# krzyz/topo-renderer

Measured on AMD Instinct MI355X. Metric: panorama Mpix/s, higher is better.
Workload: dtype f32; 1 GPU; c4: 10x10 deg COP90-shaped mosaic (100 tiles of 1200x1200 f32), 16384x4096 panorama = 8 sectors of 2048x4096, view_mode 0; frames_in_flight=1

## Files before the change

topo-renderer_amd/__init__.py:

```python
from __future__ import annotations

import ctypes as C
import math
import os
import subprocess

import numpy as np

from . import panorama, synth

_HERE = os.path.dirname(os.path.abspath(__file__))
LIB_PATH = os.environ.get("TOPO_HIP_LIB") or os.path.join(_HERE, "libtopo_hip.so")
HEADER_PATH = os.path.join(os.path.dirname(_HERE), "include", "topo_hip.h")
TEST_HEADER_PATH = os.path.join(os.path.dirname(_HERE), "include", "topo_hip_test.h")

TOPO_OK = 0
TOPO_ERR_INVALID, TOPO_ERR_UNSUPPORTED, TOPO_ERR_HIP, TOPO_ERR_NOT_FOUND, TOPO_ERR_CAPACITY = -1, -2, -3, -4, -5
FORMAT_RGBA8_UNORM_SRGB, FORMAT_BGRA8_UNORM_SRGB, FORMAT_RGBA8_UNORM, FORMAT_BGRA8_UNORM = 1, 2, 3, 4
TIMING_SLOTS = 9
TIMING_NAMES = ("clear", "cull", "raster", "occlusion", "raster_big", "resolve", "total", "load", "load_tables")

NEAR, FAR = 50.0, 500000.0
N_SECTORS = 8
HORIZON_SKY, HORIZON_INCOMPLETE = -1, -2
HORIZON_DTYPE = np.dtype([("row", "<i4"), ("depth", "<f4"), ("lat_deg", "<i4"), ("lon_deg", "<i4"), ("cell_x", "<u4"), ("cell_y", "<u4"),
                          ("fan", "<u4"), ("_reserved", "<u4")])
GROUND_TERRAIN, GROUND_SKY, GROUND_OUTSIDE, GROUND_INCOMPLETE, GROUND_DEGENERATE = 1, 0, -1, -2, -3
GROUND_DTYPE = np.dtype([("lon_deg", "<f8"), ("lat_deg", "<f8"), ("height_m", "<f4"), ("range_m", "<f4"), ("depth", "<f4"), ("kind", "<i4"),
                         ("tile_lat_deg", "<i4"), ("tile_lon_deg", "<i4"), ("cell_x", "<u4"), ("cell_y", "<u4"), ("tri", "<u4"), ("fan", "<u4"),
                         ("w1", "<f4"), ("w2", "<f4")])
GROUND_QUERY_DTYPE = np.dtype([("view", "<u4"), ("x", "<u4"), ("y", "<u4"), ("_reserved", "<u4")])
RAY_HIT, RAY_MISS, RAY_INVALID = 1, 0, -1
SUN_NONE, SUN_LIT, SUN_AWAY, SUN_SHADOW = 0, 1, 2, 3
RAY_DTYPE = np.dtype([("origin", "<f8", 3), ("dir", "<f8", 3), ("t_min", "<f8"), ("t_max", "<f8")])
RAY_HIT_DTYPE = np.dtype([("t", "<f8"), ("lon_deg", "<f8"), ("lat_deg", "<f8"), ("height_m", "<f4"), ("kind", "<i4"), ("tile_lat_deg", "<i4"),
                          ("tile_lon_deg", "<i4"), ("cell_x", "<u4"), ("cell_y", "<u4"), ("tri", "<u4"), ("front", "<u4"), ("w1", "<f4"), ("w2", "<f4")])
UNWRAP_EQUIRECTANGULAR, UNWRAP_CYLINDRICAL = 0, 1
UNWRAP_NEAREST, UNWRAP_BILINEAR = 0, 1
UNWRAP_PARAMS_DTYPE = np.dtype([("projection", "<u4"), ("filter", "<u4"), ("out_w", "<u4"), ("out_h", "<u4"), ("az0_deg", "<f8"), ("az_span_deg", "<f8"),
                                ("el_top_deg", "<f8"), ("el_bottom_deg", "<f8")])


class TopoError(RuntimeError):
    def __init__(self, code, msg):
        super().__init__(f"topo_hip error {code}: {msg}")
        self.code = code


def build(verbose: bool = False) -> str:
    subprocess.check_call(["make", "-C", os.path.join(_HERE, "csrc"), "all"] + ([] if verbose else ["-s"]))
    return LIB_PATH


_lib = None


def _preload_torch_hip_runtime():
    import importlib.util
    try:
        spec = importlib.util.find_spec("torch")
    except (ImportError, ValueError):
        spec = None
    if spec and spec.submodule_search_locations:
        cand = os.path.join(list(spec.submodule_search_locations)[0], "lib", "libamdhip64.so")
        if os.path.exists(cand):
            C.CDLL(cand, mode=C.RTLD_GLOBAL)


def lib():
    global _lib
    if _lib is None:
        if not os.path.exists(LIB_PATH):
            raise ImportError(f"{LIB_PATH} is missing -- run `python -c 'import __graft_entry__ as g; g.build()'` "
                              "(there is no Python/CPU fallback for the render path)")
        _preload_torch_hip_runtime()
        L = C.CDLL(LIB_PATH)
        vp, u32, i32, f32, sz = C.c_void_p, C.c_uint32, C.c_int32, C.c_float, C.c_size_t
        sigs = {
            "topo_create": (C.c_int, [C.POINTER(vp), C.c_int, u32, u32, u32]),
            "topo_destroy": (None, [vp]),
            "topo_last_error": (C.c_char_p, [vp]),
            "topo_add_terrain": (C.c_int, [vp, i32, i32, vp, u32, u32, vp, vp, vp]),
            "topo_add_terrain_device": (C.c_int, [vp, i32, i32, vp, u32, u32, vp, vp, vp]),
            "topo_unload_terrain": (C.c_int, [vp, i32, i32]),
            "topo_update": (C.c_int, [vp, u32, u32, vp, vp]),
            "topo_render": (C.c_int, [vp, vp, sz, vp, sz]),
            "topo_recompute_normals": (C.c_int, [vp]),
            "topo_render_views_device": (C.c_int, [vp, u32, vp, u32, u32, vp, sz, sz, vp, sz, sz]),
            "topo_set_stream": (C.c_int, [vp, vp]),
            "topo_synchronize": (C.c_int, [vp]),
            "topo_set_normals_lds_rows": (C.c_int, [vp, C.c_int]),
            "topo_debug_set_queue_caps": (C.c_int, [vp, u32, u32]),
            "topo_debug_far_phase_launched": (C.c_int, [vp, vp]),
            "topo_debug_set_tile_prefilter": (C.c_int, [vp, i32]),
            "topo_debug_cull_pairs": (C.c_int, [vp, vp]),
            "topo_pin_host_buffer": (C.c_int, [vp, vp, sz]),
            "topo_unpin_host_buffer": (C.c_int, [vp, vp]),
            "topo_get_timings": (C.c_int, [vp, vp]),
            "topo_get_timing_history": (C.c_int, [vp, C.c_uint32, vp, vp]),
            "topo_get_counters": (C.c_int, [vp, vp]),
            "topo_set_occlusion_split": (C.c_int, [vp, f32]),
            "topo_set_timing_slots": (C.c_int, [vp, u32]),
            "topo_read_normals": (C.c_int, [vp, i32, i32, vp]),
            "topo_read_tile_tables": (C.c_int, [vp, i32, i32, vp, vp, vp, vp]),
            "topo_probe_sincos": (C.c_int, [vp, vp, vp, vp, sz]),
            "topo_probe_div": (C.c_int, [vp, i32, vp, vp, vp, sz]),
            "topo_set_pipeline_depth": (C.c_int, [vp, i32]),
            "topo_join": (C.c_int, [vp]),
            "topo_frame_status": (C.c_int, [vp, vp]),
            "topo_overlay_lines": (C.c_int, [vp, vp, u32, vp, u32, f32, vp, sz]),
            "topo_overlay_lines_device": (C.c_int, [vp, vp, u32, vp, u32, f32, vp, sz]),
            "topo_overlay_glyphs": (C.c_int, [vp, vp, u32, C.c_float, vp, u32, u32, vp, sz]),
            "topo_overlay_glyphs_device": (C.c_int, [vp, vp, u32, C.c_float, vp, u32, u32, vp, sz]),
            "topo_change_location_plan": (None, [f32, f32, f32, vp, u32, vp, u32, vp, vp, u32, vp]),
            "topo_change_location": (C.c_int, [vp, f32, f32, f32, vp, u32, vp, vp]),
            "topo_comm_unique_id": (C.c_int, [vp]),
            "topo_comm_init": (C.c_int, [C.POINTER(vp), C.c_int, vp, C.c_int, C.c_int]),
            "topo_comm_from_nccl": (C.c_int, [C.POINTER(vp), vp, C.c_int, C.c_int]),
            "topo_comm_destroy": (None, [vp]),
            "topo_panorama_sector_range": (None, [C.c_int, C.c_int, vp, vp]),
            "topo_panorama_slots": (u32, [C.c_int, u32, u32, vp, u32]),
            "topo_render_panorama": (C.c_int, [vp, vp, vp, f32, f32, u32, u32, f32, f32, i32, vp, vp]),
            "topo_render_batch": (C.c_int, [vp, u32, vp, vp, vp, f32, u32, u32, i32, vp, vp]),
            "topo_visible_peaks": (C.c_int, [vp, u32, vp, vp, vp]),
            "topo_visible_peaks_device": (C.c_int, [vp, vp, u32, u32, vp, sz, u32, vp, vp, vp]),
            "topo_camera_uniforms": (None, [vp, f32, f32, f32, f32, f32, f32, f32, i32, vp]),
            "topo_terrain_uniforms": (None, [vp, vp, vp, u32, u32, vp]),
            "topo_geometry_transform": (None, [f32, f32, f32, vp]),
            "topo_dist_from_depth": (f32, [f32]),
            "topo_pad_256": (u32, [u32]),
            "topo_synth_tile": (None, [i32, i32, u32, u32, u32, vp]),
            "topo_locations_range": (u32, [f32, f32, f32, vp, u32]),
            "topo_coordinate_transform": (C.c_int, [vp, u32, vp, u32, vp, vp, vp, vp]),
            "topo_geotiff_info": (C.c_int, [vp, sz, vp, vp, vp, vp, vp]),
            "topo_sector_fov_y": (f32, [u32, u32, u32]),
            "topo_panorama_uniforms": (None, [vp, f32, f32, u32, u32, f32, f32, i32, u32, vp]),
            "topo_render_device": (C.c_int, [vp, vp, sz, vp, sz]),
            "topo_geotiff_decode": (C.c_int, [vp, vp, sz, vp, sz]),
            "topo_add_terrain_geotiff": (C.c_int, [vp, i32, i32, vp, sz]),
            "topo_to_model": (None, [vp, vp, vp, f32, f32, vp]),
            "topo_to_raster": (None, [vp, vp, vp, f32, f32, vp]),
            "topo_height_value_at": (C.c_int, [vp, u32, u32, vp, vp, vp, C.c_double, C.c_double, vp]),
            "topo_viewshed_enable": (C.c_int, [vp, i32]),
            "topo_viewshed_reset": (C.c_int, [vp]),
            "topo_viewshed_read": (C.c_int, [vp, i32, i32, vp, sz, vp]),
            "topo_debug_viewshed_stats": (C.c_int, [vp, vp]),
            "topo_horizon_shape": (C.c_int, [vp, vp, vp, vp]),
            "topo_horizon_read": (C.c_int, [vp, u32, u32, vp, sz]),
            "topo_horizon_device": (C.c_int, [vp, u32, u32, vp, sz]),
            "topo_pixel_angles": (None, [vp, u32, u32, u32, vp, vp]),
            "topo_ground_read": (C.c_int, [vp, u32, vp, vp]),
            "topo_ground_device": (C.c_int, [vp, u32, vp, vp]),
            "topo_ground_map_device": (C.c_int, [vp, u32, u32, vp, sz, sz]),
            "topo_raycast_read": (C.c_int, [vp, u32, vp, vp]),
            "topo_raycast_device": (C.c_int, [vp, u32, vp, vp]),
            "topo_sunlit_map_device": (C.c_int, [vp, u32, u32, vp, vp, sz, sz]),
            "topo_sun_direction": (None, [C.c_double, C.c_double, C.c_double, C.c_double, vp]),
            "topo_unwrap_device": (C.c_int, [vp, vp, u32, vp, u32, u32, vp, sz, sz, vp, sz, sz, vp, sz, vp, sz, vp, sz]),
            "topo_unwrap_xy": (None, [vp, u32, vp, vp]),
        }
        for name, (res, args) in sigs.items():
            fn = getattr(L, name)
            fn.restype = res
            fn.argtypes = args
        L._topo_symbols = tuple(sigs)
        _lib = L
    return _lib


def _p(a):
    return a.ctypes.data_as(C.c_void_p)



def camera_uniforms(eye, yaw, pitch, fov_y, width, height, sun_theta_deg, sun_phi_deg, view_mode=0) -> np.ndarray:
    out = np.zeros(40, dtype=np.float32)
    e = np.ascontiguousarray(eye, dtype=np.float32)
    lib().topo_camera_uniforms(_p(e), yaw, pitch, fov_y, width, height, sun_theta_deg, sun_phi_deg, view_mode, _p(out))
# ... 305 lines not shown

    def overlay_glyphs(self, glyphs, atlas: np.ndarray, rgba: np.ndarray, depth: float = 100.0 / 4096.0) -> np.ndarray:
        g = np.ascontiguousarray(glyphs)
        a = np.ascontiguousarray(atlas, dtype=np.uint8)
        assert rgba.dtype == np.uint8 and rgba.flags.c_contiguous
        self._check(lib().topo_overlay_glyphs(self._h, _p(g), g.nbytes // 28, depth, _p(a), a.shape[1], a.shape[0], _p(rgba), rgba.strides[0]))
        return rgba

    def overlay_glyphs_device(self, glyphs, atlas: np.ndarray, rgba_ptr: int, rgba_pitch: int, depth: float = 100.0 / 4096.0):
        g = np.ascontiguousarray(glyphs)
        a = np.ascontiguousarray(atlas, dtype=np.uint8)
        self._check(lib().topo_overlay_glyphs_device(self._h, _p(g), g.nbytes // 28, depth, _p(a), a.shape[1], a.shape[0], C.c_void_p(rgba_ptr), rgba_pitch))

    def change_location(self, latitude: float, longitude: float, range_dist: float = 100_000.0):
        rq = np.zeros((4096, 2), np.int32)
        nr, nu = C.c_uint32(), C.c_uint32()
        self._check(lib().topo_change_location(self._h, latitude, longitude, range_dist, _p(rq), 4096, C.byref(nr), C.byref(nu)))
        return [(int(a), int(b)) for a, b in rq[:nr.value]], int(nu.value)

    def render_panorama(self, comm, eye, yaw0, sector_w, sector_h, sun_theta_deg, sun_phi_deg, strip_ptr: int, depth_ptr: int = 0,
                        view_mode: int = 0, pitch: float = 0.0):
        e = np.ascontiguousarray(eye, dtype=np.float32)
        self._check(lib().topo_render_panorama(self._h, comm._h if comm is not None else None, _p(e), yaw0, pitch, sector_w, sector_h,
                                               sun_theta_deg, sun_phi_deg, view_mode, C.c_void_p(strip_ptr),
                                               C.c_void_p(depth_ptr) if depth_ptr else None))

    def render_batch(self, eyes, yaw0s, suns_theta_phi_deg, sector_w, sector_h, rgba_ptr: int, depth_ptr: int = 0, view_mode: int = 0,
                     pitch: float = 0.0):
        e = np.ascontiguousarray(eyes, dtype=np.float32).reshape(-1, 3)
        y = np.ascontiguousarray(yaw0s, dtype=np.float32).reshape(-1)
        sn = np.ascontiguousarray(suns_theta_phi_deg, dtype=np.float32).reshape(-1, 2)
        assert len(e) == len(y) == len(sn)
        self._check(lib().topo_render_batch(self._h, len(e), _p(e), _p(y), _p(sn), pitch, sector_w, sector_h, view_mode,
                                            C.c_void_p(rgba_ptr), C.c_void_p(depth_ptr) if depth_ptr else None))

    def render_views_device(self, uniforms_list, width, height, rgba_ptr: int, rgba_view_stride: int, rgba_pitch: int,
                            depth_ptr: int = 0, depth_view_stride: int = 0, depth_pitch: int = 0):
        if isinstance(uniforms_list, np.ndarray) and uniforms_list.dtype == np.uint8 and uniforms_list.ndim == 2:
            us = np.ascontiguousarray(uniforms_list)
            assert us.shape[1] == 160
        else:
            us = np.ascontiguousarray(np.stack([np.ascontiguousarray(u).view(np.uint8).reshape(160) for u in uniforms_list]))
        self._check(lib().topo_render_views_device(self._h, len(us), _p(us), width, height,
                                                   C.c_void_p(rgba_ptr), rgba_view_stride, rgba_pitch,
                                                   C.c_void_p(depth_ptr) if depth_ptr else None, depth_view_stride, depth_pitch))

    def set_stream(self, hip_stream: int):
        self._check(lib().topo_set_stream(self._h, C.c_void_p(hip_stream) if hip_stream else None))

    def set_pipeline_depth(self, depth: int):
        self._check(lib().topo_set_pipeline_depth(self._h, depth))

    def join(self):
        self._check(lib().topo_join(self._h))

    def synchronize(self):
        self._check(lib().topo_synchronize(self._h))

    def frame_status(self) -> dict:
        out = np.zeros(4, np.uint32)
        self._check(lib().topo_frame_status(self._h, _p(out)))
        return {"status": int(out[0]), "big_overflow": bool(out[0] & 1), "rare_overflow": bool(out[0] & 2), "bounds_violation": bool(out[0] & 4),
                "bounds_site": int(out[1]), "bounds_value": int(out[2]) | (int(out[3]) << 32)}

    def set_normals_lds_rows(self, rows: int):
        self._check(lib().topo_set_normals_lds_rows(self._h, rows))

    def debug_set_queue_caps(self, big_cap: int, rare_cap: int):
        self._check(lib().topo_debug_set_queue_caps(self._h, big_cap, rare_cap))

    def debug_far_phase_launched(self) -> bool:
        out = np.zeros(1, np.int32)
        self._check(lib().topo_debug_far_phase_launched(self._h, _p(out)))
        return bool(out[0])

    def debug_set_tile_prefilter(self, on: bool):
        self._check(lib().topo_debug_set_tile_prefilter(self._h, 1 if on else 0))

    def debug_cull_pairs(self) -> tuple:
        out = np.zeros(2, np.uint32)
        self._check(lib().topo_debug_cull_pairs(self._h, _p(out)))
        return int(out[0]), int(out[1])

    def timings(self) -> dict:
        out = np.zeros(TIMING_SLOTS, np.float32)
        self._check(lib().topo_get_timings(self._h, _p(out)))
        return {k: float(v) for k, v in zip(TIMING_NAMES, out) if k != "_"}

    def timing_history(self, n_frames: int) -> list:
        out, n = np.zeros((max(1, n_frames), 7), np.float32), C.c_uint32(0)
        self._check(lib().topo_get_timing_history(self._h, n_frames, _p(out), C.byref(n)))
        return [{k: float(v) for k, v in zip(TIMING_NAMES[:7], row)} for row in out[:n.value]]

    def counters(self) -> dict:
        out = np.zeros(6, np.uint32)
        self._check(lib().topo_get_counters(self._h, _p(out)))
        return {"blocks_rastered": int(out[0]) + int(out[5]), "big_items": int(out[1]), "status": int(out[2]), "rare_items": int(out[3]),
                "near_blocks": int(out[0]), "far_tested": int(out[4]), "far_survived": int(out[5])}

    def set_timing_slots(self, names=None, total=True):
        mask = 0x3F if names is None else sum(1 << TIMING_NAMES.index(n) for n in names)
        if not total:
            mask |= 0x80
        self._check(lib().topo_set_timing_slots(self._h, mask))

    def set_occlusion_split(self, metres: float):
        self._check(lib().topo_set_occlusion_split(self._h, metres))

    def read_tile_tables(self, lat_deg, lon_deg) -> dict:
        w, h = self.tile_size
        n = C.c_uint32(0)
        self._check(lib().topo_read_tile_tables(self._h, lat_deg, lon_deg, None, None, None, C.byref(n)))
        minmax, trig, bounds = np.empty((n.value, 2), np.float32), np.empty((w + h, 2), np.float32), np.empty(n.value * 17, np.float64)
        self._check(lib().topo_read_tile_tables(self._h, lat_deg, lon_deg, _p(minmax), _p(trig), _p(bounds), C.byref(n)))
        return {"minmax": minmax, "trig": trig, "bounds": bounds}

    def read_normals(self, lat_deg, lon_deg) -> np.ndarray:
        w, h = self.tile_size
        out = np.empty((h, w, 4), np.uint8)
        self._check(lib().topo_read_normals(self._h, lat_deg, lon_deg, _p(out)))
        return out

    def visible_peaks(self, peaks_xyz: np.ndarray):
        pk = np.ascontiguousarray(peaks_xyz, dtype=np.float32).reshape(-1, 3)
        n = pk.shape[0]
        vis = np.zeros(n, np.uint8)
        xy = np.zeros((n, 2), np.uint32)
        self._check(lib().topo_visible_peaks(self._h, n, _p(pk), _p(vis), _p(xy)))
        return vis.astype(bool), xy

    def visible_peaks_device(self, uniforms, width, height, depth_ptr, depth_pitch, n, peaks_ptr, visible_ptr, xy_ptr):
        u = np.ascontiguousarray(uniforms).view(np.uint8)
        self._check(lib().topo_visible_peaks_device(self._h, _p(u), width, height, C.c_void_p(depth_ptr), depth_pitch, n,
                                                    C.c_void_p(peaks_ptr), C.c_void_p(visible_ptr), C.c_void_p(xy_ptr)))

    def viewshed_enable(self, on: bool = True):
        self._check(lib().topo_viewshed_enable(self._h, 1 if on else 0))

    def viewshed_reset(self):
        self._check(lib().topo_viewshed_reset(self._h))

    def viewshed(self, lat_deg, lon_deg) -> np.ndarray:
        if self.tile_size is None:
            raise TopoError(TOPO_ERR_NOT_FOUND, "no tile loaded")
        w, h = self.tile_size
        out = np.zeros((h - 1, w - 1), np.uint8)
        n = C.c_uint64(0)
        self._check(lib().topo_viewshed_read(self._h, lat_deg, lon_deg, _p(out), w - 1, C.byref(n)))
        if int(out.sum()) != n.value:
            raise TopoError(TOPO_ERR_INVALID, f"viewshed count {n.value} differs from the mask's {int(out.sum())} cells")
        return out.astype(bool)

    def debug_viewshed_stats(self) -> dict:
        out = np.zeros(3, np.uint64)
        self._check(lib().topo_debug_viewshed_stats(self._h, _p(out)))
        return {"terrain_keys": int(out[0]), "updates": int(out[1]), "atomics": int(out[2])}

    def horizon_shape(self):
        n, w, h = C.c_uint32(), C.c_uint32(), C.c_uint32()
        self._check(lib().topo_horizon_shape(self._h, C.byref(n), C.byref(w), C.byref(h)))
        return int(n.value), int(w.value), int(h.value)

    def horizon(self, first_view: int = 0, n_views: int = None) -> np.ndarray:
        total, w, _ = self.horizon_shape()
        n = total - first_view if n_views is None else n_views
        out = np.zeros((max(n, 0), w), HORIZON_DTYPE)
# ... 69 lines not shown
```

topo-renderer_amd/csrc/kernels_frame.h:

```cpp
#pragma once

#include "kernels_common.h"

namespace topo {
namespace {

__device__ __forceinline__ void clear_body(uint64_t* __restrict__ vis, uint8_t* __restrict__ dirty, size_t n, uint32_t* __restrict__ counters,
                                           uint32_t* __restrict__ zero, uint32_t block, uint32_t n_blocks) {
    if (block == 0)
        for (uint32_t i = threadIdx.x; i < kCounterWords; i += 256) zero[i] = 0;
    const uint32_t lane = threadIdx.x & 63;
    const size_t nseg = (n + 63) >> 6, wave = (size_t)block * 4 + (threadIdx.x >> 6), nwave = (size_t)n_blocks * 4;
    for (size_t g = wave * 64; g < nseg; g += nwave * 64) {
        const bool mine = g + lane < nseg && dirty[g + lane] != 0;
        uint64_t todo = __ballot(mine);
        if (mine) dirty[g + lane] = 0;
        while (todo) {
            const size_t seg = g + (size_t)__builtin_ctzll(todo);
            todo &= todo - 1;
            if (TOPO_CHK(counters, seg * 64 + lane < ((n + 63) & ~(size_t)63), 3u, seg * 64 + lane))
                vis[seg * 64 + lane] = kVisClear;
        }
    }
}
// ... 172 lines not shown
__global__ __launch_bounds__(256) void k_clear_cull(FrameParams P, uint32_t n_cull_blocks, uint32_t n_clear_blocks, uint32_t* __restrict__ zero, ViewPack pack,
                                                    uint32_t pack_words, uint32_t wgs_per_pair, CullPairs pairs) {
    if (pack_words) {
        const auto src = kernarg<uint32_t>(offsetof(ClearCullArgs, pack));
        if (blockIdx.x == 0 && threadIdx.x < pack_words) const_cast<uint32_t*>(reinterpret_cast<const uint32_t*>(P.views))[threadIdx.x] = src[threadIdx.x];
        P.views = (const ViewDev*)(const void*)src;
    }
    const uint32_t total = n_cull_blocks + n_clear_blocks;
    const uint32_t before = (uint32_t)((uint64_t)blockIdx.x * n_clear_blocks / total), upto = (uint32_t)((uint64_t)(blockIdx.x + 1u) * n_clear_blocks / total);
    if (upto > before) clear_body(P.vis, P.dirty, (size_t)P.n_views * P.W * P.H, P.counters, zero, before, n_clear_blocks);
    else cull_body(P, blockIdx.x - before, kernarg<uint32_t>(offsetof(ClearCullArgs, pairs)), wgs_per_pair);
}

#ifndef TOPO_OCC_ROWS
#define TOPO_OCC_ROWS 4
#endif
constexpr uint32_t kOccRows = TOPO_OCC_ROWS;
__global__ __launch_bounds__(256) void k_occlusion(FrameParams P) {
    if (blockIdx.x == 0 && threadIdx.x == 0) {
        P.counters[kCtrBigStart] = P.counters[kCtrBig];
        P.counters[kCtrRareStart] = P.counters[kCtrRare];
    }
    const uint32_t lane = threadIdx.x & 63;
    const uint32_t wave_global = blockIdx.x * 4 + __builtin_amdgcn_readfirstlane(threadIdx.x >> 6), wave_count = gridDim.x * 4;
    static_assert(kFarLists == 64, "one sub-list per lane");
    uint32_t incl = min(P.counters[far_list_counter(lane)], P.far_sub_cap);
#pragma unroll
    for (int o = 1; o < 64; o <<= 1) {
        const uint32_t up = (uint32_t)__shfl_up((int)incl, o);
        if ((int)lane >= o) incl += up;
    }
    const uint32_t count = (uint32_t)__shfl((int)incl, 63);
    if (blockIdx.x == 0 && threadIdx.x == 0) P.counters[kCtrFarTested] = count;
    auto entry = [&](uint32_t g) -> const FarItem& {
        const uint32_t q = (uint32_t)__popcll(__ballot(incl <= g));
        const uint32_t start = q ? (uint32_t)__shfl((int)incl, (int)q - 1) : 0u;
        return P.far[(size_t)q * P.far_sub_cap + (g - start)];
    };
    if (count == 0) return;
    FarItem fi_next = entry(wave_global < count ? wave_global : 0u);
    for (uint32_t item = wave_global; item < count; item += wave_count) {
        const FarItem fi = fi_next;
        fi_next = entry(item + wave_count < count ? item + wave_count : item);
        const uint64_t* vis = P.vis + (size_t)(fi.view_rank >> 16) * P.W * P.H;
        bool visible = false;
        for (uint32_t x = fi.x0; x <= fi.x1 && !visible; x += 64) {
            const uint32_t px = min(x + lane, (uint32_t)fi.x1);
            for (uint32_t y = fi.y0; y <= fi.y1; y += kOccRows) {
                uint32_t d[kOccRows];
#pragma unroll
                for (uint32_t k = 0; k < kOccRows; ++k) {
                    const size_t at = (size_t)min(y + k, (uint32_t)fi.y1) * P.W + px;
                    d[k] = TOPO_CHK(P.counters, at < (size_t)P.W * P.H && (fi.view_rank >> 16) < P.n_views, 6u, at) ? (uint32_t)(vis[at] >> 32) : 0u;
                }
                bool open = false;
#pragma unroll
                for (uint32_t k = 0; k < kOccRows; ++k) open |= d[k] >= fi.zmin_bits;
                if (__any(open)) { visible = true; break; }
            }
        }
        if (visible && lane == 0) {
            const uint32_t blk = fi.block, by = blk / P.bx_count;
            const uint32_t cell_rows = min(kBCY, P.tile_h - 1 - by * kBCY);
            const uint32_t strip = P.near_strip, n = (cell_rows + strip - 1) / strip;
            const uint32_t base = atomicAdd(&P.counters[kCtrFarSurvived], n);
            for (uint32_t k = 0; k < n; ++k)
                if (base + k < P.near_cap)
                    P.work2[base + k] = WorkItem{fi.view_rank, blk | ((strip * k) << 24) | (min(strip, cell_rows - strip * k) << 28)};
        }
    }
}



__device__ __forceinline__ void raster_box(const TriSetup& ts, const Vis& vis, int32_t W, uint32_t id,
                                           int32_t px0, int32_t px1, int32_t py0, int32_t py1) {
    for (int32_t py = py0; py <= py1; ++py)
        for (int32_t px = px0; px <= px1; ++px) {
            float z, b[3];
            if (triangle_pixel(ts, px, py, z, b)) vis_min(vis, (size_t)py * W + px, vis_key(z, id));
        }
}

__device__ bool enqueue_big(const FrameParams& P, uint32_t view, uint32_t id, const SVert& s0, const SVert& s1, const SVert& s2,
                            int32_t px0, int32_t px1, int32_t py0, int32_t py1) {
    const int32_t rx0 = px0 >> 6, rx1 = px1 >> 6, ry0 = py0 >> 6, ry1 = py1 >> 6;
    const uint32_t n = (uint32_t)((rx1 - rx0 + 1) * (ry1 - ry0 + 1));
    const uint32_t base = atomicAdd(&P.counters[kCtrBig], n);
    BigItem it;
    it.view = view;
    it.id = id;
    it.X[0] = s0.X; it.X[1] = s1.X; it.X[2] = s2.X;
    it.Y[0] = s0.Y; it.Y[1] = s1.Y; it.Y[2] = s2.Y;
    it.z[0] = s0.z; it.z[1] = s1.z; it.z[2] = s2.z;
    if (base >= P.big_cap || n > P.big_cap - base) {
        atomicOr(&P.counters[kCtrStatus], kStatusBigOverflow);
        it.id = kNoTri;
        it.region = 0;
        for (uint32_t k = base; k < P.big_cap && k - base < n; ++k) P.big[k] = it;
        return false;
    }
    uint32_t k = base;
    for (int32_t ry = ry0; ry <= ry1; ++ry)
        for (int32_t rx = rx0; rx <= rx1; ++rx) {
            it.region = ((uint32_t)ry << 16) | (uint32_t)rx;
            if (TOPO_CHK(P.counters, k < P.big_cap && rx >= 0 && ry >= 0 && rx * 64 < P.W && ry * 64 < P.H, 7u, k)) P.big[k] = it;
            ++k;
        }
    return true;
}

__device__ __forceinline__ void enqueue_rare(const FrameParams& P, uint32_t view, uint32_t draw) {
    const uint32_t slot = atomicAdd(&P.counters[kCtrRare], 1u);
    if (slot < P.rare_cap) P.rare[slot] = RareItem{view, draw};
    else atomicOr(&P.counters[kCtrStatus], kStatusRareOverflow);
}

#ifndef TOPO_FRAG_CAP
#define TOPO_FRAG_CAP 128
#endif
constexpr uint32_t kFragCap = TOPO_FRAG_CAP;
struct FragList {
    uint32_t count;
    uint32_t pix[kFragCap];
    uint64_t key[kFragCap];
};

#ifndef TOPO_INLANE_ROWS
#define TOPO_INLANE_ROWS 5
#endif
#ifndef TOPO_INLANE_COLS
#define TOPO_INLANE_COLS 24
#endif
constexpr int32_t kInlaneRows = TOPO_INLANE_ROWS, kInlaneCols = TOPO_INLANE_COLS;

__device__ __forceinline__ void frag_push(FragList& fl, const Vis& vis, uint32_t pix, uint64_t key) {
    const uint32_t slot = atomicAdd(&fl.count, 1u);
    if (slot < kFragCap) {
        fl.pix[slot] = pix;
        fl.key[slot] = key;
    } else {
        vis_min(vis, pix, key);
    }
}

constexpr uint32_t kTriCap = 128;
struct TriList {
    int32_t X0[kTriCap], Y0[kTriCap], X1[kTriCap], Y1[kTriCap], X2[kTriCap], Y2[kTriCap];
    float z0[kTriCap], z1[kTriCap], z2[kTriCap];
    uint32_t id[kTriCap];
};

__device__ __forceinline__ bool classify_small(const FrameParams& P, const SVert& s0, const SVert& s1, const SVert& s2, uint32_t view,
                                               uint32_t id) {
    const int32_t X0 = s0.X, Y0 = s0.Y, X1 = s1.X, Y1 = s1.Y, X2 = s2.X, Y2 = s2.Y;
    const int32_t mnx = min(X0, min(X1, X2)), mxx = max(X0, max(X1, X2));
    const int32_t mny = min(Y0, min(Y1, Y2)), mxy = max(Y0, max(Y1, Y2));
    if ((mxx - mnx) >= (1 << 14) || (mxy - mny) >= (1 << 14)) {
        enqueue_rare(P, view, id >> 1);
        return false;
    }
    const int32_t area2 = __mul24(X1 - X0, Y2 - Y0) - __mul24(Y1 - Y0, X2 - X0);
    if (area2 >= 0) return false;
    const int32_t px0 = max((mnx + 127) >> 8, 0), px1 = min((mxx - 128) >> 8, P.W - 1);
    const int32_t py0 = max((mny + 127) >> 8, 0), py1 = min((mxy - 128) >> 8, P.H - 1);
    if (px0 > px1 || py0 > py1) return false;
    if (py1 - py0 >= kInlaneRows || px1 - px0 >= kInlaneCols) {
        if (!enqueue_big(P, view, id, s0, s1, s2, px0, px1, py0, py1)) enqueue_rare(P, view, id >> 1);
        return false;
    }
    return true;
}


__device__ __forceinline__ uint32_t tri_push(TriList& tl, uint32_t n, bool push, const SVert& s0, const SVert& s1, const SVert& s2,
                                             uint32_t id, uint32_t* vis_counters) {
    const uint64_t mask = __ballot(push);
    if (push) {
        const uint32_t slot = n + __popcll(mask & ((1ull << (threadIdx.x & 63)) - 1ull));
        if (!TOPO_CHK(vis_counters, slot < kTriCap, 8u, slot)) return n;
        tl.X0[slot] = s0.X; tl.Y0[slot] = s0.Y; tl.X1[slot] = s1.X; tl.Y1[slot] = s1.Y; tl.X2[slot] = s2.X; tl.Y2[slot] = s2.Y;
        tl.z0[slot] = s0.z; tl.z1[slot] = s1.z; tl.z2[slot] = s2.z;
        tl.id[slot] = id;
    }
    return n + (uint32_t)__popcll(mask);
}

__device__ __forceinline__ uint32_t tri_drain(TriList& tl, FragList& fl, const Vis& vis, int32_t W, int32_t H, uint32_t n,
                                              bool flush) {
    const uint32_t lane = threadIdx.x & 63;
    const uint32_t take = min(n, 64u), base = n - take;
    if (lane < take) {
// ... 47 lines not shown
        }
        const auto view_proj = const_space(P.views[view_idx].proj);
        const uint32_t blk_id = wi.block & 0xFFFFFFu, strip_first = (wi.block >> 24) & 15u, strip_rows = wi.block >> 28;
        const uint32_t bx = blk_id % P.bx_count, by = blk_id / P.bx_count;
        const uint32_t x0 = bx * kBCX, y0 = by * kBCY + strip_first;
        const uint32_t nrows = min(strip_rows ? strip_rows + 1 : kVY, P.tile_h - y0);
        const uint32_t ncx = min(kBCX, P.tile_w - 1 - x0);
        const uint32_t vx = x0 + lane;
        const bool vcol = lane < kVX && vx < P.tile_w;
        const Vis vis = view_vis(P, view_idx);
        float proj[16];
#pragma unroll
        for (int q = 0; q < 16; ++q) proj[q] = view_proj[q];
        if (lane == 0) fl.count = 0;
        float slo, clo, lat_s = 0.0f, lat_c = 0.0f;
        sincos_f(vertex_lon(t, vcol ? vx : x0), slo, clo);
        if (lane < nrows) sincos_f(vertex_lat(t, y0 + lane), lat_s, lat_c);
        const auto hcol = TOPO_GLOBAL_F32(t.heights) + (size_t)y0 * P.tile_w + (vcol ? vx : x0);
        (void)TOPO_CHK(P.counters, rank < P.n_tiles && view_idx < P.n_views && y0 + nrows <= P.tile_h && (vcol ? vx : x0) < P.tile_w && nrows >= 1u, 9u,
                       ((uint64_t)y0 << 32) | x0);
        float h0 = hcol[0];
        float h1 = nrows > 1 ? hcol[(size_t)1 * P.tile_w] : 0.0f;
        float h2 = nrows > 2 ? hcol[(size_t)2 * P.tile_w] : 0.0f;
        float h3 = nrows > 3 ? hcol[(size_t)3 * P.tile_w] : 0.0f;
        SVert prev;
        prev.X = 0; prev.Y = 0; prev.z = 0.0f; prev.flag = kVtxNear;
        for (uint32_t r = 0; r < nrows; ++r) {
            const float h = h0;
            h0 = h1; h1 = h2; h2 = h3;
            if (r + 4 < nrows) h3 = hcol[(size_t)(r + 4) * P.tile_w];
            const float sla = __shfl(lat_s, (int)r), cla = __shfl(lat_c, (int)r);
            SVert cur;
            cur.X = 0; cur.Y = 0; cur.z = 0.0f; cur.flag = kVtxNear;
            if (vcol) {
                const f3 p = world_from_sincos(h, sla, cla, slo, clo);
                float clip[4];
                mat4_point(proj, p.x, p.y, p.z, clip);
                clip_to_screen(clip, (float)P.W, (float)P.H, cur);
            }
            if (r > 0) {
                const SVert cc = shfl_down1(prev), d = shfl_down1(cur);
                bool live = lane < ncx;
                if (live && (prev.flag | cur.flag | cc.flag | d.flag) == kVtxOk) {
                    const int32_t qx0 = min(min(prev.X, cur.X), min(cc.X, d.X)), qx1 = max(max(prev.X, cur.X), max(cc.X, d.X));
                    const int32_t qy0 = min(min(prev.Y, cur.Y), min(cc.Y, d.Y)), qy1 = max(max(prev.Y, cur.Y), max(cc.Y, d.Y));
                    const int32_t bx0 = max((qx0 + 127) >> 8, 0), bx1 = min((qx1 - 128) >> 8, P.W - 1);
                    const int32_t by0 = max((qy0 + 127) >> 8, 0), by1 = min((qy1 - 128) >> 8, P.H - 1);
                    live = bx0 <= bx1 && by0 <= by1;
                }
                const SVert &a = prev, &b = cur;
                const uint32_t i = x0 + lane, j = y0 + r - 1;
                const bool even = ((i + j) & 1u) == 0;
                const uint32_t tri0 = (i * (P.tile_h - 1) + j) * 2;
#pragma unroll
                for (uint32_t k = 0; k < 2; ++k) {
                    const SVert& s0 = k == 0 ? a : d;
                    const SVert& s1 = k == 0 ? b : cc;
                    const SVert& s2 = k == 0 ? (even ? d : cc) : (even ? a : b);
                    const uint32_t draw = rank * P.tris_per_tile + tri0 + k;
                    bool push = false;
                    if (live) {
                        const int fg = s0.flag | s1.flag | s2.flag;
                        if (fg == kVtxOk) {
                            push = classify_small(P, s0, s1, s2, view_idx, draw << 1);
                        } else if (fg & kVtxNear) {
                            const int nnear = (s0.flag == kVtxNear) + (s1.flag == kVtxNear) + (s2.flag == kVtxNear);
                            if (nnear != 3) enqueue_rare(P, view_idx, draw);
                        }
                    }
                    ntri = tri_push(tl, ntri, push, s0, s1, s2, draw << 1, P.counters);
                    if (ntri >= 64) ntri = tri_drain(tl, fl, vis, P.W, P.H, ntri, false);
                }
            }
            prev = cur;
        }
        while (ntri > 0) ntri = tri_drain(tl, fl, vis, P.W, P.H, ntri, true);
        const uint32_t nfrag = min(fl.count, kFragCap);
        for (uint32_t f = lane; f < nfrag; f += 64) vis_min(vis, fl.pix[f], fl.key[f]);
        if (lane == 0) fl.count = 0;
    }
}

constexpr uint32_t kCoopRegions = 24;
__global__ __launch_bounds__(256) void k_raster_rare(FrameParams P) {
    uint32_t count = P.counters[kCtrRare];
    if (count > P.rare_cap) count = P.rare_cap;
    const uint32_t lane = threadIdx.x & 63;
    for (uint32_t item = P.counters[kCtrRareStart] + blockIdx.x * blockDim.x + threadIdx.x; item < count; item += gridDim.x * blockDim.x) {
        const RareItem ri = P.rare[item];
        const uint32_t rank = fastdiv(ri.draw, P.div_tris), tri = ri.draw - rank * P.tris_per_tile;
        if (!TOPO_CHK(P.counters, rank < P.n_tiles && ri.view < P.n_views, 10u, ri.draw)) continue;
        const Vis vis = view_vis(P, ri.view);
        for (uint32_t fan = 0; fan < 2; ++fan) {
            ResolvedTri r;
            const bool has = resolve_triangle(P.tiles[rank], P.tile_w, P.div_hm1, P.tile_h - 1, P.views[ri.view], P.W, P.H, tri, fan, r);
            const TriSetup& ts = r.ts;
            const uint32_t id = (ri.draw << 1) | fan;
            const int32_t nx = has ? ts.px1 - ts.px0 + 1 : 0, ny = has ? ts.py1 - ts.py0 + 1 : 0;
            const bool small = nx <= 4 && ny <= 4;
            const int32_t rx0 = has ? ts.px0 >> 6 : 0, rx1 = has ? ts.px1 >> 6 : 0, ry0 = has ? ts.py0 >> 6 : 0, ry1 = has ? ts.py1 >> 6 : 0;
            const uint32_t rw = (uint32_t)(rx1 - rx0 + 1), n_regions = rw * (uint32_t)(ry1 - ry0 + 1);
            const bool coop = has && !small && n_regions >= kCoopRegions && rw <= 256u;
            bool in_lane = has && small;
            if (has && !small && !coop) in_lane = !enqueue_big(P, ri.view, id, r.s[0], r.s[1], r.s[2], ts.px0, ts.px1, ts.py0, ts.py1);
            uint64_t jobs = __ballot(coop);
            if (jobs) {
                const uint64_t act = __ballot(true);
                const uint32_t n_act = (uint32_t)__popcll(act), mine = (uint32_t)__popcll(act & ((1ull << lane) - 1ull));
                while (jobs) {
                    const int L = __builtin_ctzll(jobs);
                    jobs &= jobs - 1ull;
                    auto from = [&](int32_t v) { return __builtin_amdgcn_readlane(v, L); };
                    BigItem it;
                    it.view = (uint32_t)from((int32_t)ri.view);
                    it.id = (uint32_t)from((int32_t)id);
#pragma unroll
                    for (int k = 0; k < 3; ++k) {
                        it.X[k] = from(r.s[k].X);
                        it.Y[k] = from(r.s[k].Y);
                        it.z[k] = wave_lane(r.s[k].z, L);
                    }
                    const int32_t jx0 = from(rx0), jy0 = from(ry0);
                    const uint32_t jw = (uint32_t)from((int32_t)rw), n = (uint32_t)from((int32_t)n_regions);
                    uint32_t base = 0;
                    if ((int)lane == L) base = atomicAdd(&P.counters[kCtrBig], n);
                    base = (uint32_t)from((int32_t)base);
                    if (base >= P.big_cap || n > P.big_cap - base) {
                        if ((int)lane == L) { atomicOr(&P.counters[kCtrStatus], kStatusBigOverflow); in_lane = true; }
                        it.id = kNoTri;
                        it.region = 0;
                        for (uint32_t k = mine; k < n && base + k < P.big_cap; k += n_act) P.big[base + k] = it;
                        continue;
                    }
                    const uint32_t magic = region_split_magic(jw);
                    for (uint32_t k = mine; k < n; k += n_act) {
                        const uint32_t q = region_split_row(k, jw, n, magic);
                        const int32_t ry = jy0 + (int32_t)q, rx = jx0 + (int32_t)(k - q * jw);
                        it.region = ((uint32_t)ry << 16) | (uint32_t)rx;
                        if (TOPO_CHK(P.counters, base + k < P.big_cap && rx >= 0 && ry >= 0 && rx * 64 < P.W && ry * 64 < P.H, 7u, base + k)) P.big[base + k] = it;
                    }
                }
            }
            if (in_lane) raster_box(ts, vis, P.W, id, ts.px0, ts.px1, ts.py0, ts.py1);
        }
    }
}

__global__ __launch_bounds__(256) void k_raster_big(FrameParams P) {
    __shared__ uint8_t s_rows[4][64];
    uint32_t count = P.counters[kCtrBig];
    if (count > P.big_cap) count = P.big_cap;
    const uint32_t lane = threadIdx.x & 63, wave = __builtin_amdgcn_readfirstlane(threadIdx.x >> 6);
    s_rows[wave][lane] = 0;
    const uint32_t wave_global = blockIdx.x * 4 + wave, wave_count = gridDim.x * 4;
    for (uint32_t item = P.counters[kCtrBigStart] + wave_global; item < count; item += wave_count) {
        BigItem bi;
        {
            const BigItem& g = P.big[item];
            bi.view = wave_first(g.view); bi.id = wave_first(g.id); bi.region = wave_first(g.region);
#pragma unroll
            for (int k = 0; k < 3; ++k) { bi.X[k] = wave_first(g.X[k]); bi.Y[k] = wave_first(g.Y[k]); bi.z[k] = wave_first(g.z[k]); }
        }
        if (bi.id == kNoTri) continue;
        const Vis vis = view_vis(P, bi.view);
        const int32_t rx = (int32_t)(bi.region & 0xFFFFu), ry = (int32_t)(bi.region >> 16);
        if (!TOPO_CHK(P.counters, bi.view < P.n_views && rx * 64 < P.W && ry * 64 < P.H, 11u, bi.region)) continue;
        uint8_t* const rows = s_rows[wave];
        if (spans_fit_int32(bi.X[0], bi.Y[0], bi.X[1], bi.Y[1], bi.X[2], bi.Y[2])) {
            big_medium_lane(bi.X, bi.Y, bi.z, bi.id, P.W, P.H, rx, ry, lane, [&](const uint32_t pix[4], const uint64_t key[4], const int32_t py[4]) {
#pragma unroll
                for (int k = 0; k < 4; ++k)
                    if (key[k] != kVisClear) {
                        vis_min_unmarked(vis, pix[k], key[k]);
                        rows[py[k] & 63] = 1;
                    }
            });
        } else {
            big_giant_lane(bi.X, bi.Y, bi.z, bi.id, P.W, P.H, rx, ry, lane, [&](size_t pix, uint64_t key, int32_t py) {
                vis_min_unmarked(vis, pix, key);
                rows[py & 63] = 1;
            });
        }
        if (rows[lane]) {
            rows[lane] = 0;
            const int32_t y = ry * 64 + (int32_t)lane, x0 = rx * 64, x1 = min(rx * 64 + 63, P.W - 1);
            const size_t first = (size_t)(vis.p - vis.base) + (size_t)y * P.W;
            const size_t s0 = (first + x0) >> 6, s1 = (first + x1) >> 6;
            if (TOPO_CHK(P.counters, y < P.H && s1 < (((size_t)P.n_views * P.W * P.H + 63) >> 6), 14u, s1)) {
                vis.dirty[s0] = 1;
                if (s1 != s0) vis.dirty[s1] = 1;
            }
        }
    }
}

}

__global__ __launch_bounds__(256) void k_put_views(ViewPack pack, uint32_t n_words, uint32_t* __restrict__ dst) {
    static_assert(sizeof(ViewPack) % 4 == 0 && sizeof(ViewPack) / 4 <= 256, "one word per lane");
    const auto src = kernarg<uint32_t>();
    if (threadIdx.x < n_words) dst[threadIdx.x] = src[threadIdx.x];
}

}
```

topo-renderer_amd/csrc/terrain_renderer.cpp:

```cpp
#include "terrain_renderer.hpp"

#include "geotiff.hpp"

#include <algorithm>
#include <atomic>
#include <thread>
#include <cmath>
#include <cstdio>
#include <cstring>

namespace topo {

namespace {

struct Switches {
    static int env(const char* name, int unset) { return getenv(name) ? atoi(getenv(name)) : unset; }
    const bool views_by_copy = env("TOPO_VIEWS_BY_COPY", 0) != 0;
    const bool views_in_cull = env("TOPO_VIEWS_IN_CULL", 1) != 0;
    const bool status_by_copy = env("TOPO_STATUS_BY_COPY", 0) != 0;
    const bool far_skip = env("TOPO_FAR_SKIP", 1) != 0;
    const bool events_by_marker = env("TOPO_EVENTS_BY_MARKER", 0) != 0;
    const bool fuse_clear_cull = env("TOPO_FUSE_CLEAR_CULL", 1) != 0;
    const bool tile_prefilter = env("TOPO_TILE_PREFILTER", 1) != 0;
    const int near_strip = env("TOPO_NEAR_STRIP", 0);
};
const Switches& switches() { static const Switches s; return s; }

bool is_linear(uint32_t format) { return format == TOPO_FORMAT_RGBA8_UNORM || format == TOPO_FORMAT_BGRA8_UNORM; }
bool is_bgra(uint32_t format) { return format == TOPO_FORMAT_BGRA8_UNORM_SRGB || format == TOPO_FORMAT_BGRA8_UNORM; }

constexpr int kTimingSlots = 6;
constexpr uint32_t kStagesOfSlot[kTimingSlots] = {1u << kStClear, 1u << kStCull, (1u << kStRasterNear) | (1u << kStRasterFar), 1u << kStOcclusion,
                                                  (1u << kStRareBigNear) | (1u << kStRareBigFar), 1u << kStResolve};
constexpr uint32_t stage_events(int stage) { return 3u << stage; }
constexpr uint32_t kLastEvent = 1u << kNumStages, kTotalEvents = 1u | kLastEvent;

}

int TerrainRenderer::fail(int code, const std::string& msg) {
    err_ = msg;
    return code;
}

int TerrainRenderer::hip_fail(hipError_t e, const char* what) {
    err_ = std::string(what) + ": " + hipGetErrorString(e);
    return TOPO_ERR_HIP;
}

int TerrainRenderer::bind_device() {
    TOPO_HIP_TRY(hipSetDevice(device_));
    return TOPO_OK;
}

int TerrainRenderer::create(TerrainRenderer** out, int device, uint32_t w, uint32_t h, uint32_t format, std::string* err) {
    *out = nullptr;
    if (w == 0 || h == 0) { *err = "target size must be non-zero"; return TOPO_ERR_INVALID; }
    if (format < TOPO_FORMAT_RGBA8_UNORM_SRGB || format > TOPO_FORMAT_BGRA8_UNORM) {
        *err = "colour format must be Rgba8UnormSrgb, Bgra8UnormSrgb, Rgba8Unorm or Bgra8Unorm";
        return TOPO_ERR_UNSUPPORTED;
    }
    int count = 0;
    hipError_t e = hipGetDeviceCount(&count);
    if (e != hipSuccess || count == 0) {
        *err = std::string("no HIP device: ") + (e != hipSuccess ? hipGetErrorString(e) : "device count is 0") +
               " (this library has no CPU fallback)";
        return TOPO_ERR_HIP;
    }
    if (device < 0 || device >= count) { *err = "hip_device out of range"; return TOPO_ERR_INVALID; }
    TerrainRenderer* r = new TerrainRenderer();
    r->device_ = device;
    r->W_ = w;
    r->H_ = h;
    r->format_ = format;
    if (r->init() != TOPO_OK) {
        *err = "HIP initialisation failed: " + r->err_;
        delete r;
        return TOPO_ERR_HIP;
    }
    *out = r;
    return TOPO_OK;
}

int TerrainRenderer::init() {
    TOPO_HIP_TRY(hipSetDevice(device_));
    TOPO_HIP_TRY(hipStreamCreate(&own_stream_.h));
    stream_ = own_stream_;
    tile_prefilter_ = switches().tile_prefilter;
    for (auto& e : load_ev_) TOPO_HIP_TRY(hipEventCreate(&e.h));
    return init_ctx(ctx_[0], false);
}

TerrainRenderer::~TerrainRenderer() {
    (void)hipSetDevice(device_);
    if (stream_) (void)hipStreamSynchronize(stream_);
    for (auto& c : ctx_)
        if (c.stream) (void)hipStreamSynchronize(c.stream);
}

int TerrainRenderer::ensure(hipStream_t s, DeviceBuffer& b, size_t need) {
    if (need <= b.cap) return TOPO_OK;
    if (b.p) {
        TOPO_HIP_TRY(hipStreamSynchronize(s));
        TOPO_HIP_TRY(hipFree(b.p));
        b.p = nullptr;
        b.cap = 0;
    }
    TOPO_HIP_TRY(hipMalloc(&b.p, need));
// ... 322 lines not shown
}

static bool far_phase_empty(const topo_uniforms* views, uint32_t n, const std::map<GeoKey, Tile>& tiles, float* split_m) {
    double bound = 0.0;
    for (uint32_t i = 0; i < n && bound >= 0.0; ++i) {
        const float* m = views[i].camera_proj;
        const double wn = std::sqrt((double)m[3] * m[3] + (double)m[7] * m[7] + (double)m[11] * m[11]);
        for (const auto& kv : tiles) {
            const double* s = kv.second.centres;
            const double w_far = (double)m[3] * s[0] + (double)m[7] * s[1] + (double)m[11] * s[2] + (double)m[15] + s[3] * wn;
            if (!(s[3] >= 0.0) || !(w_far < 1e30)) { bound = -1.0; break; }
            bound = std::max(bound, w_far);
        }
    }
    if (!(bound >= 0.0 && bound + 2.0 < (double)*split_m * (4.0 / 3.0))) return false;
    *split_m = std::max(*split_m, (float)(bound + 2.0));
    return true;
}

static bool fused_clear_cull(const FrameParams& p) { return switches().fuse_clear_cull && p.n_tiles != 0; }

int TerrainRenderer::render_frame(FrameCtx& c, hipStream_t stream, uint32_t n, const topo_uniforms* views, uint32_t w, uint32_t h,
                                  const OutputParams& out, const ResolveSlot* slots, uint32_t n_slots,
                                  const std::function<int(uint32_t, hipStream_t)>* after_slot) {
    if (n == 0) return fail(TOPO_ERR_INVALID, "null/empty argument");
    if (const char* e = submission_error(n, w, h)) return fail(TOPO_ERR_INVALID, e);
    latest_ctx_ = -1;
    FrameParams p{};
    if (int rc = grow_frame_buffers(c, stream, n, w, h, p)) return rc;
    ViewPack pack{};
    bool pack_in_cull = false;
    if (int rc = stage_views(c, stream, views, p, pack, &pack_in_cull)) return rc;
    fill_params(c, p);
    last_far_phase_ = p.split_m > 0.0f && !(switches().far_skip && far_phase_empty(views, n, tiles_, &p.split_m));
    const CullList cull = cull_pairs(views, p);
    if (int rc = queue_frame(c, stream, p, pack_in_cull ? &pack : nullptr, cull, last_far_phase_, out, slots, n_slots, after_slot)) return rc;
    record_submission(c, p, views);
    TOPO_HIP_TRY(hipGetLastError());
    return TOPO_OK;
}

TerrainRenderer::CullList TerrainRenderer::cull_pairs(const topo_uniforms* views, const FrameParams& p) {
    const size_t all = (size_t)p.n_views * p.n_tiles;
    last_cull_pairs_[0] = last_cull_pairs_[1] = (uint32_t)all;
    CullList list{nullptr, 0};
    if (!tile_prefilter_ || all == 0 || all > 65536) return list;
    const uint32_t kept = tile_prefilter(views, p.n_views, tile_spheres().data(), p.n_tiles, cull_codes_, kMaxCullPairs);
    if (kept > kMaxCullPairs) return list;
    last_cull_pairs_[0] = kept;
    list.codes = cull_codes_;
    list.n = kept;
    return list;
}

int TerrainRenderer::grow_frame_buffers(FrameCtx& c, hipStream_t stream, uint32_t n, uint32_t w, uint32_t h, FrameParams& p) {
    p.n_views = n;
    p.n_tiles = (uint32_t)tiles_.size();
    p.W = (int32_t)w;
    p.H = (int32_t)h;
    p.bx_count = p.n_tiles ? (tile_w_ - 1 + kBCX - 1) / kBCX : 0;
    p.by_count = p.n_tiles ? (tile_h_ - 1 + kBCY - 1) / kBCY : 0;
    const size_t pixels = (size_t)n * w * h;
    const size_t work_cap = (size_t)n * p.n_tiles * p.bx_count * p.by_count;
    p.big_cap = big_cap_cfg_ ? big_cap_cfg_ : (1u << 22);
    p.rare_cap = rare_cap_cfg_ ? rare_cap_cfg_ : (rare_cap_auto_ ? (uint32_t)rare_cap_auto_ : (1u << 22));
    if (work_cap >= (1ull << 30)) return fail(TOPO_ERR_CAPACITY, "too many raster blocks in one submission");
    if (pixels >= (1ull << 32)) return fail(TOPO_ERR_CAPACITY, "more than 2^32 pixels in one submission");
    const size_t vis_keys = (pixels + 63) & ~(size_t)63;
    if (vis_keys * 8 > c.d_vis.cap) {
        if (int rc = ensure(stream, c.d_vis, vis_keys * 8)) return rc;
        if (int rc = ensure(stream, c.d_dirty, vis_keys / 64 + 64)) return rc;
        TOPO_HIP_TRY(hipMemsetAsync(c.d_dirty.p, 1, c.d_dirty.cap, stream));
    }
    if (int rc = ensure(stream_, d_views_, sizeof(ViewDev) * kMaxViewsPerSlot * kViewSlots)) return rc;
    const int strip_env = switches().near_strip;
    p.near_strip = strip_env >= 1 && strip_env <= 15 ? (uint32_t)strip_env : (work_cap <= 64 * 1024 ? 1u : 2u);
    const size_t near_cap = (size_t)((kBCY + p.near_strip - 1) / p.near_strip) * work_cap;
    if (int rc = ensure(stream, c.d_work, (near_cap ? near_cap : 1) * sizeof(WorkItem))) return rc;
    if (int rc = ensure(stream, c.d_work2, (near_cap ? near_cap : 1) * sizeof(WorkItem))) return rc;
    const size_t far_sub_cap = (cull_workgroups_max(n, p.n_tiles, p.bx_count * p.by_count) + kFarLists - 1) / kFarLists * 256;
    if (int rc = ensure(stream, c.d_far, (far_sub_cap ? far_sub_cap * kFarLists : 1) * sizeof(FarItem))) return rc;
    if (int rc = ensure(stream, c.d_big, p.big_cap * sizeof(BigItem))) return rc;
    if (int rc = ensure(stream, c.d_rare, p.rare_cap * sizeof(RareItem))) return rc;
    if (!c.d_counters.p) {
        if (int rc = ensure(stream, c.d_counters, 2 * kCounterWords * sizeof(uint32_t))) return rc;
        TOPO_HIP_TRY(hipMemsetAsync(c.d_counters.p, 0, 2 * kCounterWords * sizeof(uint32_t), stream));
    }
    if (int rc = ensure_pinned(c.h_status, kStatusRing * kStatusWords * sizeof(uint32_t))) return rc;
    if (c.submitted - c.checked == kStatusRing) {
        if (c.last_stream) TOPO_HIP_TRY(hipStreamSynchronize(c.last_stream));
        overflow_pending_ |= fold_frames(c);
    }
    c.last_stream = stream;
    c.pending = pipeline_depth_ > 1;
    p.work_cap = (uint32_t)work_cap;
    p.far_sub_cap = (uint32_t)far_sub_cap;
    p.near_cap = (uint32_t)near_cap;
    return TOPO_OK;
}

int TerrainRenderer::stage_views(FrameCtx& c, hipStream_t stream, const topo_uniforms* views, FrameParams& p, ViewPack& pack, bool* pack_in_cull) {
    const uint32_t n = p.n_views;
    if (n > kMaxViewsPerSlot) return fail(TOPO_ERR_INVALID, "too many views in one submission");
    static_assert(kViewSlots % kMaxPipeline == 0, "every frame context has its own share of the slots");
    const int slot = (int)(&c - ctx_) * (kViewSlots / kMaxPipeline) + (int)(c.frames % (kViewSlots / kMaxPipeline));
    ViewDev* d_slot = d_views_.as<ViewDev>() + (size_t)slot * kMaxViewsPerSlot;
    p.views = d_slot;
    auto fill_views = [&](ViewDev* vd) {
        for (uint32_t i = 0; i < n; ++i) {
            memcpy(vd[i].proj, views[i].camera_proj, sizeof vd[i].proj);
            vd[i].cam_x = views[i].camera_pos[0];
            vd[i].cam_y = views[i].camera_pos[1];
            memcpy(vd[i].sun, views[i].sun_direction, sizeof vd[i].sun);
            vd[i].view_mode = views[i].view_mode;
        }
    };
    const bool packed = n <= kPackViews && !switches().views_by_copy;
    *pack_in_cull = packed && fused_clear_cull(p) && switches().views_in_cull;
    if (packed) {
        fill_views(pack.v);
        if (!*pack_in_cull) launch_put_views(pack, n, d_slot, stream);
        return TOPO_OK;
    }
    if (!view_ev_[kViewSlots - 1]) {
        if (int rc = ensure_pinned(h_views_, sizeof(ViewDev) * kMaxViewsPerSlot * kViewSlots)) return rc;
        for (auto& e : view_ev_)
            if (!e) TOPO_HIP_TRY(hipEventCreateWithFlags(&e.h, hipEventDisableTiming));
    }
    if (view_used_[slot]) TOPO_HIP_TRY(hipEventSynchronize(view_ev_[slot]));
    ViewDev* vd = h_views_.as<ViewDev>() + (size_t)slot * kMaxViewsPerSlot;
    fill_views(vd);
    TOPO_HIP_TRY(hipMemcpyAsync(d_slot, vd, n * sizeof(ViewDev), hipMemcpyHostToDevice, stream));
    TOPO_HIP_TRY(hipEventRecord(view_ev_[slot], stream));
    view_used_[slot] = true;
    return TOPO_OK;
}

void TerrainRenderer::fill_params(FrameCtx& c, FrameParams& p) {
    p.tiles = d_tiles_.as<const TileDev>();
    p.vis = c.d_vis.as<uint64_t>();
    p.dirty = c.d_dirty.as<uint8_t>();
    p.work = c.d_work.as<WorkItem>();
    p.counters = c.d_counters.as<uint32_t>() + (c.frames & 1u) * kCounterWords;
#ifdef TOPO_BOUNDS_CHECK
    p.status_out = nullptr;
#else
    p.status_out = switches().status_by_copy ? nullptr : c.status_words(c.submitted);
#endif
    p.big = c.d_big.as<BigItem>();
    p.rare = c.d_rare.as<RareItem>();
    p.far = c.d_far.as<FarItem>();
    p.work2 = c.d_work2.as<WorkItem>();
    p.split_m = occlusion_split_m_;
    p.tile_w = tile_w_;
    p.tile_h = tile_h_;
    p.tris_per_tile = p.n_tiles ? 2u * (tile_w_ - 1) * (tile_h_ - 1) : 8u;
    p.div_tris = fastdiv_make(p.tris_per_tile);
    p.div_hm1 = fastdiv_make(p.n_tiles ? tile_h_ - 1 : 2u);
    p.rblocks_x = ((uint32_t)p.W + kResolveBlockW - 1) / kResolveBlockW;
    p.rblocks_view = p.rblocks_x * (((uint32_t)p.H + kResolveBlockH - 1) / kResolveBlockH);
    p.div_rblocks_x = fastdiv_make(p.rblocks_x > 1 ? p.rblocks_x : 2u);
    p.div_rblocks_view = fastdiv_make(p.rblocks_view > 1 ? p.rblocks_view : 2u);
    float thresh[256];
    for (int i = 0; i < 256; ++i) thresh[i] = bits_f(TOPO_SRGB_THRESH_BITS[i]);
    p.linear_target = is_linear(format_) ? 1u : 0u;
    p.bgra = is_bgra(format_) ? 1u : 0u;
    p.sky_c8 = (p.linear_target ? to_unorm8(0.0f) | (to_unorm8(0.71f) << 8) | (to_unorm8(0.885f) << 16)
                                : srgb_encode(thresh, 0.0f) | (srgb_encode(thresh, 0.71f) << 8) | (srgb_encode(thresh, 0.885f) << 16)) |
               (to_unorm8(1.0f) << 24);
}

int TerrainRenderer::queue_frame(FrameCtx& c, hipStream_t stream, FrameParams& p, const ViewPack* pack_in_cull, const CullList& cull, bool far_phase, const OutputParams& out,
                                 const ResolveSlot* slots, uint32_t n_slots, const std::function<int(uint32_t, hipStream_t)>* after_slot) {
    const uint32_t n = p.n_views, w = (uint32_t)p.W, h = (uint32_t)p.H;
    uint32_t* const counters_next = c.d_counters.as<uint32_t>() + ((c.frames & 1u) ^ 1u) * kCounterWords;
    uint32_t ev_need = timing_total_ ? kTotalEvents : 0u;
    for (int sl = 0; sl < kTimingSlots; ++sl)
        for (int st = 0; st < kNumStages; ++st)
            if ((timing_slots_ & (1u << sl)) && (kStagesOfSlot[sl] & (1u << st))) ev_need |= stage_events(st);
    const bool pixelize = post_.pixelize_n < 99.99999f;
    const bool own_times = !switches().events_by_marker && !pixelize && (ev_need & ~(kTotalEvents | stage_events(kStResolve))) == 0;
    FrameCtx::TimedFrame& tf = c.timed_frames[c.frames++ % kEvRing];
    tf.recorded = ev_need;
    tf.slots = timing_slots_;
    tf.frame = ++frame_seq_;
    auto mark = [&](int i, bool may_be_own = false) { return (ev_need >> i & 1u) && !(may_be_own && own_times) ? hipEventRecord(tf.ev[i], stream) : hipSuccess; };
    auto own = [&](int i) -> hipEvent_t { return (ev_need >> i & 1u) && own_times ? (hipEvent_t)tf.ev[i] : nullptr; };
    TOPO_HIP_TRY(mark(kStClear, true));
    const hipEvent_t ev_first = own(kStClear);
    const bool fuse = fused_clear_cull(p);
    if (fuse) launch_clear_cull(p, counters_next, stream, ev_first, pack_in_cull, n, cull.codes, cull.n);
    else launch_clear(p, counters_next, stream, ev_first);
    TOPO_HIP_TRY(mark(kStCull));
    if (!fuse) launch_cull(p, stream, cull.codes, cull.n);
    TOPO_HIP_TRY(mark(kStRasterNear));
    launch_raster(p, 0, stream);
    TOPO_HIP_TRY(mark(kStRareBigNear));
    launch_raster_rare(p, stream);
    launch_raster_big(p, stream);
    TOPO_HIP_TRY(mark(kStOcclusion));
    if (far_phase) launch_occlusion(p, stream);
    TOPO_HIP_TRY(mark(kStRasterFar));
    if (far_phase) launch_raster(p, 1, stream);
    TOPO_HIP_TRY(mark(kStRareBigFar));
    if (far_phase) {
        launch_raster_rare(p, stream);
        launch_raster_big(p, stream);
    }
    TOPO_HIP_TRY(mark(kStResolve, true));
    const hipEvent_t ev_rstart = own(kStResolve), ev_rstop = own(kNumStages);
    OutputParams kout = out;
    if (pixelize) {
        if (n_slots) return fail(TOPO_ERR_UNSUPPORTED, "the pixelise branch is not available on the slot-by-slot (multi-GPU) path");
        const size_t img = (size_t)w * h * 4;
        if (int rc = ensure(stream, c.d_pre_rgba, img * n)) return rc;
        if (!out.depth)
            if (int rc = ensure(stream, c.d_pre_depth, img * n)) return rc;
        kout.rgba = c.d_pre_rgba.as<uint8_t>();
        kout.rgba_view_stride = img;
        kout.rgba_pitch = (size_t)w * 4;
        if (!out.depth) { kout.depth = c.d_pre_depth.as<float>(); kout.depth_view_stride = img; kout.depth_pitch = (size_t)w * 4; }
        p.post_off = 1;
    }
    if (n_slots == 0) {
        p.rblock_first = 0;
        p.rblock_count = p.rblocks_view * n;
        launch_resolve(p, kout, stream, ev_rstart, ev_rstop);
        if (pixelize)
            launch_post_pixelize(n, (int32_t)w, (int32_t)h, post_.viewport[0] >= 1.0f ? post_.viewport[0] : (float)w, post_.viewport[1] >= 1.0f ? post_.viewport[1] : (float)h,
                                 post_.pixelize_n, c.d_pre_rgba.as<const uint8_t>(), out, kout.depth, kout.depth_view_stride, kout.depth_pitch, p.linear_target, p.bgra, stream);
    } else {
        for (uint32_t i = 0; i < n_slots; ++i) {
            if ((uint64_t)slots[i].block_first + slots[i].block_count > (uint64_t)p.rblocks_view * n) return fail(TOPO_ERR_INVALID, "resolve slot outside the frame");
            p.rblock_first = slots[i].block_first;
            p.rblock_count = slots[i].block_count;
            launch_resolve(p, out, stream, i == 0 ? ev_rstart : nullptr, i + 1 == n_slots ? ev_rstop : nullptr);
            if (after_slot)
                if (int rc = (*after_slot)(i, stream)) return rc;
        }
    }
    if (vs_on_)
        launch_viewshed(p, d_vs_table_.as<uint32_t* const>(), d_vs_stats_.as<unsigned long long>(), stream);
    TOPO_HIP_TRY(mark(kNumStages, true));
    if (!p.status_out) TOPO_HIP_TRY(hipMemcpyAsync(c.status_words(c.submitted), p.counters, kStatusWords * sizeof(uint32_t), hipMemcpyDeviceToHost, stream));
    return TOPO_OK;
}

void TerrainRenderer::record_submission(FrameCtx& c, const FrameParams& p, const topo_uniforms* views) {
    ++c.submitted;
    c.timed = true;
    c.sub.n_views = p.n_views;
    c.sub.tile_gen = tile_gen_;
    c.sub.views.resize(p.n_views);
    for (uint32_t i = 0; i < p.n_views; ++i) {
        memcpy(c.sub.views[i].proj, views[i].camera_proj, sizeof c.sub.views[i].proj);
        memcpy(c.sub.views[i].pos, views[i].camera_pos, sizeof c.sub.views[i].pos);
        c.sub.views[i].pad_ = 0.0f;
    }
    c.sub.views_on_device = false;
    HorizonParams& q = c.sub.query;
    q.vis = p.vis;
    q.dirty = p.dirty;
    q.counters = p.counters;
    q.W = (uint32_t)p.W;
    q.H = (uint32_t)p.H;
    q.n_keys = (size_t)p.n_views * q.W * q.H;
    q.n_tiles = p.n_tiles;
    q.tris_per_tile = p.tris_per_tile;
    q.hm1 = p.n_tiles ? tile_h_ - 1 : 2u;
    q.div_tris = p.div_tris;
    q.div_hm1 = p.div_hm1;
    latest_ctx_ = (int)(&c - ctx_);
}

int TerrainRenderer::render_device(uint8_t* rgba_dev, size_t rgba_pitch, float* depth_dev, size_t depth_pitch) {
    if (!rgba_dev) return fail(TOPO_ERR_INVALID, "rgba_dev is null");
    if (!have_uniforms_) return fail(TOPO_ERR_INVALID, "topo_update has not been called");
    if (rgba_pitch < (size_t)W_ * 4 || (depth_dev && depth_pitch < (size_t)W_ * 4)) return fail(TOPO_ERR_INVALID, "pitch smaller than a row");
    return render_views_device(1, &uniforms_, W_, H_, image_output(rgba_dev, rgba_pitch, depth_dev, depth_pitch, H_));
}

int TerrainRenderer::render(uint8_t* rgba, size_t rgba_pitch, float* depth, size_t depth_pitch) {
    if (!rgba) return fail(TOPO_ERR_INVALID, "rgba_out is null");
    if (!have_uniforms_) return fail(TOPO_ERR_INVALID, "topo_update has not been called");
    if (rgba_pitch < (size_t)W_ * 4 || (depth && depth_pitch < (size_t)W_ * 4)) return fail(TOPO_ERR_INVALID, "pitch smaller than a row");
    if (int rc = bind_device()) return rc;
    const size_t row = (size_t)W_ * 4;
    if (int rc = ensure(stream_, d_out_rgba_, row * H_)) return rc;
    if (depth)
        if (int rc = ensure(stream_, d_out_depth_, row * H_)) return rc;
// ... 226 lines not shown
int TerrainRenderer::set_timing_slots(uint32_t mask) {
    timing_slots_ = mask & 0x3Fu;
    timing_total_ = !(mask & TOPO_TIMING_NO_TOTAL);
    return TOPO_OK;
}

int TerrainRenderer::set_occlusion_split(float metres) {
    if (!(metres >= 0.0f)) return fail(TOPO_ERR_INVALID, "split must be >= 0");
    occlusion_split_m_ = metres;
    return TOPO_OK;
}

int TerrainRenderer::set_queue_caps(uint32_t big_cap, uint32_t rare_cap) {
    big_cap_cfg_ = big_cap;
    rare_cap_cfg_ = (rare_cap & 0x80000000u) ? 0u : rare_cap;
    rare_cap_auto_ = (rare_cap & 0x80000000u) ? (rare_cap & 0x7FFFFFFFu) : 0u;
    return join();
}

int TerrainRenderer::frame_durations(const FrameCtx::TimedFrame& f, float out[7]) {
    for (int sl = 0; sl <= kTimingSlots; ++sl) out[sl] = 0.0f;
    for (int sl = 0; sl < kTimingSlots; ++sl)
        for (int st = 0; st < kNumStages; ++st)
            if ((f.slots & (1u << sl)) && (kStagesOfSlot[sl] & (1u << st)) && (f.recorded & stage_events(st)) == stage_events(st)) {
                float d = 0.0f;
                TOPO_HIP_TRY(hipEventElapsedTime(&d, f.ev[st], f.ev[st + 1]));
                out[sl] += d;
            }
    if ((f.recorded & kTotalEvents) == kTotalEvents) TOPO_HIP_TRY(hipEventElapsedTime(&out[kTimingSlots], f.ev[0], f.ev[kNumStages]));
    return TOPO_OK;
}

int TerrainRenderer::get_timings(float out[TOPO_TIMING_SLOTS]) {
    for (int i = 0; i < TOPO_TIMING_SLOTS; ++i) out[i] = 0.0f;
    if (int rc = bind_device()) return rc;
    FrameCtx& c = ctx_[pipeline_depth_ > 1 ? next_ctx_ : last_ctx_];
    if (c.timed && c.frames) {
        const FrameCtx::TimedFrame& f = c.timed_frames[(c.frames - 1) % kEvRing];
        if (f.recorded & kLastEvent) TOPO_HIP_TRY(hipEventSynchronize(f.ev[kNumStages]));
        else if (c.last_stream) TOPO_HIP_TRY(hipStreamSynchronize(c.last_stream));
        if (int rc = frame_durations(f, out)) return rc;
    }
    if (load_timed_) {
        TOPO_HIP_TRY(hipEventSynchronize(load_ev_[1]));
        TOPO_HIP_TRY(hipEventElapsedTime(&out[7], load_ev_[0], load_ev_[1]));
        TOPO_HIP_TRY(hipEventElapsedTime(&out[8], load_ev_[0], load_ev_[2]));
    }
    return TOPO_OK;
}

int TerrainRenderer::get_timing_history(uint32_t n_frames, float* out_ms, uint32_t* n_out) {
    *n_out = 0;
    if (!out_ms && n_frames) return fail(TOPO_ERR_INVALID, "null argument");
    if (int rc = wait_all()) return rc;
    std::vector<const FrameCtx::TimedFrame*> refs;
    for (const FrameCtx& c : ctx_)
        for (uint64_t k = 0; k < std::min<uint64_t>(c.frames, kEvRing); ++k) refs.push_back(&c.timed_frames[(c.frames - 1 - k) % kEvRing]);
    std::sort(refs.begin(), refs.end(), [](const FrameCtx::TimedFrame* a, const FrameCtx::TimedFrame* b) { return a->frame < b->frame; });
    const size_t n = std::min<size_t>(n_frames, refs.size());
    for (size_t i = 0; i < n; ++i)
        if (int rc = frame_durations(*refs[refs.size() - n + i], out_ms + 7 * i)) return rc;
    *n_out = (uint32_t)n;
    return TOPO_OK;
}

int TerrainRenderer::get_counters(uint32_t out[6]) {
    for (int i = 0; i < 6; ++i) out[i] = 0;
    FrameCtx& fc = ctx_[last_ctx_];
    if (!fc.h_status.p) return TOPO_OK;
    if (int rc = bind_device()) return rc;
    if (fc.last_stream) TOPO_HIP_TRY(hipStreamSynchronize(fc.last_stream));
    uint32_t c[kStatusWords] = {};
    if (fc.submitted) memcpy(c, fc.latest_status(), sizeof c);
    if (getenv("TOPO_DEBUG_COUNTERS")) {
        fprintf(stderr, "[topo] counters:");
        for (uint32_t i = 0; i < kStatusWords; ++i) fprintf(stderr, " %u", c[i]);
        fprintf(stderr, "\n");
    }
    static_assert(kCtrWork == 0 && kCtrFarSurvived == 5, "topo_get_counters hands out words kCtrWork .. kCtrFarSurvived");
    for (uint32_t i = kCtrWork; i <= kCtrFarSurvived; ++i) out[i] = c[i];
    return TOPO_OK;
}

int TerrainRenderer::read_normals(int32_t lat, int32_t lon, uint8_t* out) {
    Tile* t = find(lat, lon);
    if (!t) return fail(TOPO_ERR_NOT_FOUND, "no such tile");
    if (int rc = bind_device()) return rc;
    TOPO_HIP_TRY(hipStreamSynchronize(stream_));
    TOPO_HIP_TRY(hipMemcpy(out, t->d_normals, (size_t)tile_w_ * tile_h_ * 4, hipMemcpyDeviceToHost));
    return TOPO_OK;
}

int TerrainRenderer::read_tile_tables(int32_t lat, int32_t lon, float* minmax_out, float* trig_out, double* bounds_out, uint32_t* n_blocks_out) {
    Tile* t = find(lat, lon);
    if (!t) return fail(TOPO_ERR_NOT_FOUND, "no such tile");
    if (int rc = bind_device()) return rc;
    TOPO_HIP_TRY(hipStreamSynchronize(stream_));
    const uint32_t bxc = (tile_w_ - 1 + kBCX - 1) / kBCX, byc = (tile_h_ - 1 + kBCY - 1) / kBCY;
    const size_t nb = (size_t)bxc * byc;
    if (n_blocks_out) *n_blocks_out = (uint32_t)nb;
    if (minmax_out) TOPO_HIP_TRY(hipMemcpy(minmax_out, t->dev.block_minmax, nb * 2 * sizeof(float), hipMemcpyDeviceToHost));
    if (trig_out) TOPO_HIP_TRY(hipMemcpy(trig_out, t->dev.trig_lon, 2 * ((size_t)tile_w_ + tile_h_) * sizeof(float), hipMemcpyDeviceToHost));
    if (bounds_out) TOPO_HIP_TRY(hipMemcpy(bounds_out, t->dev.block_bounds, nb * 17 * sizeof(double), hipMemcpyDeviceToHost));
    return TOPO_OK;
}

int geotiff_transform(const TiffInfo& ti, float rp[2], float mp[2], float ps[2]) {
    if (ti.has_model_transformation) return TOPO_ERR_UNSUPPORTED;
    if (!ti.has_pixel_scale || !ti.has_tie_points) return TOPO_ERR_UNSUPPORTED;
    if (ti.pixel_scale.size() != 3 || ti.tie_points.size() != 6) return TOPO_ERR_INVALID;
    rp[0] = (float)ti.tie_points[0]; rp[1] = (float)ti.tie_points[1];
    mp[0] = (float)ti.tie_points[3]; mp[1] = (float)ti.tie_points[4];
    ps[0] = (float)ti.pixel_scale[0]; ps[1] = (float)ti.pixel_scale[1];
    return TOPO_OK;
}

int TerrainRenderer::geotiff_to_device(const uint8_t* bytes, size_t n, DeviceBuffer& heights, uint32_t* w, uint32_t* h, float rp[2],
                                       float mp[2], float ps[2]) {
    TiffInfo ti;
    std::string e;
    if (int rc = tiff_parse(bytes, n, ti, e)) return fail(rc, "GeoTIFF: " + e);
    if (int rc = geotiff_transform(ti, rp, mp, ps))
        return fail(rc, rc == TOPO_ERR_UNSUPPORTED ? "GeoTIFF: IncorrectGeoTags (ModelPixelScale + ModelTiepoint without ModelTransformation required)"
                                                    : "GeoTIFF: IncorrectGeoTagData (ModelPixelScale needs 3 and ModelTiepoint 6 values)");
    if (int rc = bind_device()) return rc;
    std::vector<TiffSegDev> segs;
    std::vector<uint32_t> row_seg;
    size_t total = 0;
    for (const TiffSegment& s : ti.segments) {
        TiffSegDev d{};
        d.byte_off = total; d.row0 = (uint32_t)row_seg.size();
        d.x0 = s.x0; d.y0 = s.y0; d.w = s.w; d.h = s.h;
        for (uint32_t r = 0; r < s.h; ++r) row_seg.push_back((uint32_t)segs.size());
        segs.push_back(d);
        total += (size_t)s.w * s.h * 4;
    }
    std::vector<uint8_t> staged(total);
    {
        const unsigned hw = std::thread::hardware_concurrency();
        const size_t n_thr = std::min<size_t>(segs.size(), std::min<unsigned>(hw ? hw : 1, 8));
        std::vector<int> rcs(n_thr, TOPO_OK);
        std::vector<std::string> errs(n_thr);
        std::atomic<size_t> next{0};
        auto work = [&](size_t tid) {
            for (size_t k = next++; k < segs.size(); k = next++)
                if (int rc = tiff_segment_bytes(bytes, n, ti, ti.segments[k], staged.data() + segs[k].byte_off, errs[tid])) { rcs[tid] = rc; return; }
        };
        std::vector<std::thread> pool;
        for (size_t t = 1; t < n_thr; ++t) pool.emplace_back(work, t);
        work(0);
        for (auto& th : pool) th.join();
        for (size_t t = 0; t < n_thr; ++t)
            if (rcs[t]) return fail(rcs[t], "GeoTIFF: " + errs[t]);
    }
    DeviceBuffer d_bytes, d_segs, d_rows;
    if (int rc = ensure(stream_, d_bytes, total ? total : 4)) return rc;
    if (int rc = ensure(stream_, d_segs, segs.size() * sizeof(TiffSegDev))) return rc;
    if (int rc = ensure(stream_, d_rows, row_seg.size() * sizeof(uint32_t))) return rc;
    if (int rc = ensure(stream_, heights, (size_t)ti.width * ti.height * sizeof(float))) return rc;
    TOPO_HIP_TRY(hipMemcpyAsync(d_bytes.p, staged.data(), total, hipMemcpyHostToDevice, stream_));
    TOPO_HIP_TRY(hipMemcpyAsync(d_segs.p, segs.data(), segs.size() * sizeof(TiffSegDev), hipMemcpyHostToDevice, stream_));
    TOPO_HIP_TRY(hipMemcpyAsync(d_rows.p, row_seg.data(), row_seg.size() * sizeof(uint32_t), hipMemcpyHostToDevice, stream_));
    launch_tiff_rows(d_bytes.as<uint8_t>(), d_segs.as<const TiffSegDev>(), d_rows.as<const uint32_t>(), (uint32_t)row_seg.size(), heights.as<float>(), ti.width,
                     ti.height, ti.predictor, ti.big_endian, stream_);
    TOPO_HIP_TRY(hipStreamSynchronize(stream_));
    *w = ti.width;
// ... 65 lines not shown
```

topo-renderer_amd/csrc/terrain_renderer.hpp:

```cpp
#pragma once

#include <hip/hip_runtime.h>

#include <cstdint>
#include <functional>
#include <map>
#include <string>
#include <tuple>
#include <utility>
#include <vector>

#include "../../include/topo_hip.h"
#include "host_math.hpp"
#include "topo_kernels.h"

namespace topo {

constexpr uint32_t kPanoramaSectors = 8;
struct Comm;

using GeoKey = std::tuple<int, int, int, int>;
inline GeoKey geo_key(int lat, int lon) {
    return GeoKey(lat < 0 ? -lat : lat, lat > 0 ? 1 : 0, lon < 0 ? -lon : lon, lon > 0 ? 1 : 0);
}
// ... 12 lines not shown
    Block(Block&& o) noexcept : p(std::exchange(o.p, nullptr)), cap(std::exchange(o.cap, 0)) {}
    Block& operator=(Block&& o) noexcept { if (this != &o) { reset(); p = std::exchange(o.p, nullptr); cap = std::exchange(o.cap, 0); } return *this; }
    ~Block() { reset(); }
    void reset() { if (p) (void)Free(p); p = nullptr; cap = 0; }
    template <class T> T* as() const { return static_cast<T*>(p); }
};
using DeviceBuffer = Block<hipFree>;
using PinnedBuffer = Block<hipHostFree>;
using HostRegistration = Block<hipHostUnregister>;

template <class H, hipError_t (*Destroy)(H)>
struct Handle {
    H h = nullptr;
    Handle() = default;
    Handle(Handle&& o) noexcept : h(std::exchange(o.h, nullptr)) {}
    Handle& operator=(Handle&& o) noexcept { if (this != &o) { reset(); h = std::exchange(o.h, nullptr); } return *this; }
    ~Handle() { reset(); }
    void reset() { if (h) (void)Destroy(h); h = nullptr; }
    operator H() const { return h; }
};
using Event = Handle<hipEvent_t, hipEventDestroy>;
using Stream = Handle<hipStream_t, hipStreamDestroy>;

inline OutputParams image_output(uint8_t* rgba, size_t rgba_pitch, float* depth, size_t depth_pitch, uint32_t rows) {
    return OutputParams{rgba, rgba_pitch * rows, rgba_pitch, depth, depth_pitch * rows, depth_pitch};
}

struct Tile {
    int lat = 0, lon = 0;
    uint64_t seq = 0;
    DeviceBuffer pool;
    float* d_heights = nullptr;
    uint32_t* d_normals = nullptr;
    float* d_minmax = nullptr;
    double centres[4] = {0.0, 0.0, 0.0, -1.0};
    double block_radius = -1.0;
    TileDev dev{};
    DeviceBuffer mask;
};

enum Stage { kStClear, kStCull, kStRasterNear, kStRareBigNear, kStOcclusion, kStRasterFar, kStRareBigFar, kStResolve, kNumStages };

class TerrainRenderer {
   public:
    static int create(TerrainRenderer** out, int device, uint32_t w, uint32_t h, uint32_t format, std::string* err);
    ~TerrainRenderer();

    int add_terrain(int32_t lat, int32_t lon, const float* heights, bool heights_on_device, uint32_t w, uint32_t h,
                    const float rp[2], const float mp[2], const float ps[2]);
    int unload_terrain(int32_t lat, int32_t lon);
    bool last_far_phase() const { return last_far_phase_; }
    void set_tile_prefilter(bool on) { tile_prefilter_ = on; }
    void last_cull_pairs(uint32_t out[2]) const { out[0] = last_cull_pairs_[0]; out[1] = last_cull_pairs_[1]; }
    int update(uint32_t w, uint32_t h, const topo_uniforms* u, const topo_post_uniforms* pu);
    int render(uint8_t* rgba, size_t rgba_pitch, float* depth, size_t depth_pitch);
    int render_views_device(uint32_t n, const topo_uniforms* views, uint32_t w, uint32_t h, const OutputParams& out);
    int render_device(uint8_t* rgba_dev, size_t rgba_pitch, float* depth_dev, size_t depth_pitch);
    int render_panorama(Comm* comm, const float eye[3], float yaw0, float pitch, uint32_t sector_w, uint32_t sector_h, float sun_theta_deg,
                        float sun_phi_deg, int32_t view_mode, uint8_t* strip_dev, float* depth_dev);
    int render_batch(uint32_t n_viewpoints, const float* eyes, const float* yaw0s, const float* sun_theta_phi_deg, float pitch, uint32_t sector_w,
                     uint32_t sector_h, int32_t view_mode, uint8_t* rgba_dev, float* depth_dev);
    int recompute_normals();
    int overlay_lines_device(const void* vertices, uint32_t n_vertices, const uint32_t* indices, uint32_t n_indices, float line_width, uint8_t* rgba_dev,
                             size_t rgba_pitch);
    int overlay_glyphs(const void* glyphs, uint32_t n_glyphs, float depth, const uint8_t* atlas, uint32_t atlas_w, uint32_t atlas_h, uint8_t* rgba, size_t rgba_pitch);
    int overlay_glyphs_device(const void* glyphs, uint32_t n_glyphs, float depth, const uint8_t* atlas, uint32_t atlas_w, uint32_t atlas_h, uint8_t* rgba_dev,
                              size_t rgba_pitch);
    int overlay_lines(const void* vertices, uint32_t n_vertices, const uint32_t* indices, uint32_t n_indices, float line_width, uint8_t* rgba,
                      size_t rgba_pitch);
    int change_location(float latitude, float longitude, float range_dist, std::vector<std::pair<int32_t, int32_t>>& request, uint32_t* n_unloaded);

    int set_stream(hipStream_t s);
    int synchronize();
    int set_pipeline_depth(int depth);
    int join();
    int join_frames();
    int set_normals_lds_rows(int rows);
    int set_queue_caps(uint32_t big_cap, uint32_t rare_cap);
    int pin_host_buffer(void* p, size_t bytes);
    int unpin_host_buffer(void* p);
    int get_timings(float out[TOPO_TIMING_SLOTS]);
    int get_timing_history(uint32_t n_frames, float* out_ms, uint32_t* n_out);
    int get_counters(uint32_t out[6]);
    int frame_status(uint32_t out[4]);
    int set_occlusion_split(float metres);
    int set_timing_slots(uint32_t mask);
    int read_normals(int32_t lat, int32_t lon, uint8_t* out);
    int read_tile_tables(int32_t lat, int32_t lon, float* minmax_out, float* trig_out, double* bounds_out, uint32_t* n_blocks_out);
    int geotiff_to_device(const uint8_t* bytes, size_t n, DeviceBuffer& heights, uint32_t* w, uint32_t* h, float rp[2], float mp[2], float ps[2]);
    int geotiff_decode(const uint8_t* bytes, size_t n, float* heights_out, size_t capacity);
    int add_terrain_geotiff(int32_t lat, int32_t lon, const uint8_t* bytes, size_t n);
    int probe_sincos(const float* x, float* s, float* c, size_t n);
    int probe_div(int32_t kind, const float* x, const float* y, float* out, size_t n);
    int visible_peaks(uint32_t n, const float* peaks, uint8_t* visible, uint32_t* xy);
    int visible_peaks_device(const topo_uniforms* view, uint32_t w, uint32_t h, const float* depth_dev, size_t depth_pitch,
                             uint32_t n, const float* peaks_dev, uint8_t* visible_dev, uint32_t* xy_dev);

    int viewshed_enable(bool on);
    int viewshed_reset();
    int viewshed_read(int32_t lat, int32_t lon, uint8_t* mask_out, size_t pitch, uint64_t* n_visible);
    int viewshed_stats(uint64_t out[3]);

    int horizon_shape(uint32_t* n_views, uint32_t* w, uint32_t* h);
    int horizon_read(uint32_t first_view, uint32_t n_views, topo_horizon_point* out, size_t view_stride);
    int horizon_device(uint32_t first_view, uint32_t n_views, topo_horizon_point* out_dev, size_t view_stride);

    int ground_read(uint32_t n, const topo_ground_query* queries, topo_ground_point* out);
    int ground_device(uint32_t n, const topo_ground_query* queries_dev, topo_ground_point* out_dev);
    int ground_map_device(uint32_t first_view, uint32_t n_views, float* out_dev, size_t view_stride_bytes, size_t pitch_bytes);

    int raycast_read(uint32_t n, const topo_ray* rays, topo_ray_hit* out);
    int raycast_device(uint32_t n, const topo_ray* rays_dev, topo_ray_hit* out_dev);
    int sunlit_map_device(uint32_t first_view, uint32_t n_views, const double sun_dir[3], uint8_t* out_dev, size_t view_stride_bytes, size_t pitch_bytes);

    int unwrap_device(const topo_unwrap_params* params, uint32_t n_views, const topo_uniforms* views, uint32_t src_w, uint32_t src_h, const OutputParams& src,
                      const OutputParams& out, int32_t* src_out_dev, size_t src_out_pitch);

    const char* last_error() const { return err_.c_str(); }

   private:
    TerrainRenderer() = default;
    int init();
    int fail(int code, const std::string& msg);
    int hip_fail(hipError_t e, const char* what);
    int bind_device();
    int ensure(hipStream_t s, DeviceBuffer& b, size_t need);
    int ensure_pinned(PinnedBuffer& b, size_t need);
    int wait_all();
    void collect_jobs(const Tile& nt, const std::map<GeoKey, uint32_t>& rank, std::vector<EdgeJob>& edges,
                      std::vector<CornerJob>& corners);
    int run_seam_jobs(const std::vector<EdgeJob>& edges, const std::vector<CornerJob>& corners);
    int upload_seam_jobs(const std::vector<EdgeJob>& edges, const std::vector<CornerJob>& corners);
    void launch_seam_jobs(size_t n_edges, size_t n_corners);
    void launch_load_kernels(uint32_t first, uint32_t count, hipEvent_t mid);
    std::map<GeoKey, uint32_t> ranks() const;
    Tile* find(int lat, int lon);
    int upload_tile_table();
    int overlay_upload(const void* a, size_t a_bytes, const void* b, size_t b_bytes, uint8_t** b_dev, bool* keys_fresh);
    template <class Draw> int overlay_host_image(uint8_t* rgba, size_t rgba_pitch, Draw draw);
    int alloc_mask(Tile& t);
    size_t mask_bytes() const { return (((size_t)(tile_w_ - 1) * (tile_h_ - 1) + 31) / 32) * 4; }

    int device_ = 0;
    uint32_t W_ = 0, H_ = 0;
    uint32_t format_ = TOPO_FORMAT_RGBA8_UNORM_SRGB;
    uint32_t tile_w_ = 0, tile_h_ = 0;
    topo_uniforms uniforms_{};
    topo_post_uniforms post_{{0.0f, 0.0f}, 100.0f, 0.0f};
    bool have_uniforms_ = false;
    std::map<GeoKey, Tile> tiles_;
    uint64_t next_seq_ = 1;
    bool table_dirty_ = true;
    int lds_rows_ = 0;
    uint32_t big_cap_cfg_ = 0, rare_cap_cfg_ = 0;
    uint64_t rare_cap_auto_ = 0;
    uint32_t timing_slots_ = 0x3Fu;
    bool timing_total_ = true;
    float occlusion_split_m_ = 90000.0f;

    Stream own_stream_;
    hipStream_t stream_ = nullptr;
    static constexpr int kEvRing = 32;
    static constexpr uint64_t kStatusRing = 64;
    uint64_t frame_seq_ = 0;
    Event load_ev_[3];
    bool load_timed_ = false;

    struct FrameCtx {
        Stream stream;
        struct TimedFrame {
            Event ev[kNumStages + 1];
            uint32_t recorded = 0, slots = 0;
            uint64_t frame = 0;
        } timed_frames[kEvRing];
        uint64_t frames = 0;
        Event done;
        hipStream_t last_stream = nullptr;
        bool timed = false, pending = false;
        PinnedBuffer h_status;
        uint64_t submitted = 0, checked = 0;
        uint32_t* status_words(uint64_t frame) const { return h_status.as<uint32_t>() + (frame % kStatusRing) * kStatusWords; }
        const uint32_t* latest_status() const { return status_words(submitted - 1); }
        DeviceBuffer d_vis, d_dirty;
        DeviceBuffer d_work, d_work2, d_far, d_big, d_rare, d_counters;
        DeviceBuffer d_pre_rgba, d_pre_depth;
        struct Submission {
            uint32_t n_views = 0;
            uint64_t tile_gen = 0;
            HorizonParams query{};
            std::vector<GroundView> views;
            bool views_on_device = false;
        } sub;
        DeviceBuffer d_ground_views;
    };
    static constexpr int kMaxPipeline = 4;
    FrameCtx ctx_[kMaxPipeline];
    int pipeline_depth_ = 1, next_ctx_ = 0, last_ctx_ = 0;
    int init_ctx(FrameCtx& c, bool own_stream);
    int check_frames();
    uint32_t last_status_[4] = {};
    bool fold_frames(FrameCtx& c, uint64_t end);
    bool fold_frames(FrameCtx& c) { return fold_frames(c, c.submitted); }
    bool fold_idle();
    bool fold_latest(FrameCtx& c, bool retry);
    void record_bounds(const uint32_t* words);
    bool overflow_pending_ = false;
    struct ResolveSlot { uint32_t block_first, block_count; };
    int render_frame(FrameCtx& c, hipStream_t s, uint32_t n, const topo_uniforms* views, uint32_t w, uint32_t h, const OutputParams& out,
                     const ResolveSlot* slots = nullptr, uint32_t n_slots = 0, const std::function<int(uint32_t, hipStream_t)>* after_slot = nullptr);
    int grow_frame_buffers(FrameCtx& c, hipStream_t s, uint32_t n, uint32_t w, uint32_t h, FrameParams& p);
    int stage_views(FrameCtx& c, hipStream_t s, const topo_uniforms* views, FrameParams& p, ViewPack& pack, bool* pack_in_cull);
    void fill_params(FrameCtx& c, FrameParams& p);
    struct CullList { const uint16_t* codes; uint32_t n; };
    CullList cull_pairs(const topo_uniforms* views, const FrameParams& p);
    int queue_frame(FrameCtx& c, hipStream_t s, FrameParams& p, const ViewPack* pack_in_cull, const CullList& cull, bool far_phase, const OutputParams& out,
                    const ResolveSlot* slots, uint32_t n_slots, const std::function<int(uint32_t, hipStream_t)>* after_slot);
    void record_submission(FrameCtx& c, const FrameParams& p, const topo_uniforms* views);
    int frame_durations(const FrameCtx::TimedFrame& f, float out[7]);

    DeviceBuffer d_tiles_, d_views_, d_edge_jobs_, d_corner_jobs_, d_out_rgba_, d_out_depth_;
    PinnedBuffer h_stage_;
    Event stage_ev_[8];
    std::vector<HostRegistration> pinned_;
    int download(uint8_t* dst, size_t dst_pitch, const uint8_t* src_dev, size_t row);
    static constexpr int kViewSlots = 16;
    static constexpr uint32_t kMaxViewsPerSlot = 64;
    PinnedBuffer h_views_;
    Event view_ev_[kViewSlots];
    bool view_used_[kViewSlots] = {};
    DeviceBuffer d_peaks_;
    DeviceBuffer d_proj_;
    DeviceBuffer d_overlay_geo_;
    DeviceBuffer d_overlay_keys_;
    uint32_t overlay_w_ = 0, overlay_h_ = 0;
    bool have_depth_ = false;
    uint32_t depth_w_ = 0, depth_h_ = 0;
    bool last_far_phase_ = true;
    bool tile_prefilter_ = true;
    uint16_t cull_codes_[kMaxCullPairs] = {};
    uint32_t last_cull_pairs_[2] = {0, 0};
    bool vs_on_ = false, vs_ever_ = false;
    DeviceBuffer d_vs_table_;
    DeviceBuffer d_vs_stats_;
    int latest_ctx_ = -1;
    uint64_t tile_gen_ = 0;

    struct TileTables {
        std::vector<double> spheres;
        std::vector<int32_t> ll;
        DeviceBuffer d_ll;
        DeviceBuffer d_trig, d_spheres;
        size_t trig_doubles = 0;
        uint64_t spheres_gen = ~0ull, decode_gen = ~0ull, geometry_gen = ~0ull;
    } tables_;
    enum TableLevel { kDecodeTables, kGeometryTables };
    const std::vector<double>& tile_spheres();
    int prepare_tables(TableLevel level, hipStream_t s);
    struct QueryBuffers {
        DeviceBuffer d_check, d_horizon_out, d_ground_q, d_ground_out, d_ray_in, d_ray_out, d_unwrap_tab;
        PinnedBuffer h_ray_stage;
        std::vector<double> unwrap_tab;
        std::vector<uint8_t> unwrap_key;
    } query_;
    int ensure_query_check(hipStream_t s);
    int query_fold_check();
    struct LatestSubmission { FrameCtx* c; hipStream_t s; uint32_t W, H, n_views; };
    int query_begin(uint32_t first_view, uint32_t n_views, LatestSubmission& q);
// ... 19 lines not shown
```

topo-renderer_amd/csrc/topo_capi.cpp:

```cpp
#include <cmath>
#include <cstdint>
#include <cstring>
#include <new>
#include <string>
#include <utility>
#include <vector>

#include "../../include/topo_hip_test.h"
#include "geotiff.hpp"
#include "terrain_renderer.hpp"

struct topo_ctx {
    topo::TerrainRenderer* r = nullptr;
};

namespace {
thread_local std::string g_create_error;
}

#define TOPO_GUARD(ctx)                       \
    if (!(ctx) || !(ctx)->r) return TOPO_ERR_INVALID

extern "C" {

// ... 40 lines not shown
    TOPO_CALL(ctx->r->add_terrain(lat, lon, heights, false, w, h, rp, mp, ps));
}

int topo_add_terrain_device(topo_ctx* ctx, int32_t lat, int32_t lon, const float* heights_dev, uint32_t w, uint32_t h,
                            const float rp[2], const float mp[2], const float ps[2]) {
    TOPO_GUARD(ctx);
    TOPO_CALL(ctx->r->add_terrain(lat, lon, heights_dev, true, w, h, rp, mp, ps));
}

int topo_unload_terrain(topo_ctx* ctx, int32_t lat, int32_t lon) {
    TOPO_GUARD(ctx);
    TOPO_CALL(ctx->r->unload_terrain(lat, lon));
}

int topo_update(topo_ctx* ctx, uint32_t w, uint32_t h, const topo_uniforms* u, const topo_post_uniforms* pu) {
    TOPO_GUARD(ctx);
    TOPO_CALL(ctx->r->update(w, h, u, pu));
}

int topo_render(topo_ctx* ctx, uint8_t* rgba, size_t rgba_pitch, float* depth, size_t depth_pitch) {
    TOPO_GUARD(ctx);
    TOPO_CALL(ctx->r->render(rgba, rgba_pitch, depth, depth_pitch));
}

int topo_recompute_normals(topo_ctx* ctx) {
    TOPO_GUARD(ctx);
    TOPO_CALL(ctx->r->recompute_normals());
}

int topo_render_views_device(topo_ctx* ctx, uint32_t n_views, const topo_uniforms* views, uint32_t width, uint32_t height,
                             uint8_t* rgba_dev, size_t rgba_view_stride, size_t rgba_pitch, float* depth_dev,
                             size_t depth_view_stride, size_t depth_pitch) {
    TOPO_GUARD(ctx);
    topo::OutputParams o{};
    o.rgba = rgba_dev;
    o.rgba_view_stride = rgba_view_stride;
    o.rgba_pitch = rgba_pitch;
    o.depth = depth_dev;
    o.depth_view_stride = depth_view_stride;
    o.depth_pitch = depth_pitch;
    TOPO_CALL(ctx->r->render_views_device(n_views, views, width, height, o));
}

int topo_set_stream(topo_ctx* ctx, void* hip_stream) {
    TOPO_GUARD(ctx);
    TOPO_CALL(ctx->r->set_stream((hipStream_t)hip_stream));
}

int topo_synchronize(topo_ctx* ctx) {
    TOPO_GUARD(ctx);
    TOPO_CALL(ctx->r->synchronize());
}

int topo_set_normals_lds_rows(topo_ctx* ctx, int rows) {
    TOPO_GUARD(ctx);
    return ctx->r->set_normals_lds_rows(rows);
}

int topo_debug_set_queue_caps(topo_ctx* ctx, uint32_t big_cap, uint32_t rare_cap) {
    TOPO_GUARD(ctx);
    TOPO_CALL(ctx->r->set_queue_caps(big_cap, rare_cap));
}

int topo_debug_far_phase_launched(topo_ctx* ctx, int32_t* out) {
    TOPO_GUARD(ctx);
    if (!out) return TOPO_ERR_INVALID;
    *out = ctx->r->last_far_phase() ? 1 : 0;
    return TOPO_OK;
}

int topo_debug_set_tile_prefilter(topo_ctx* ctx, int32_t on) {
    TOPO_GUARD(ctx);
    ctx->r->set_tile_prefilter(on != 0);
    return TOPO_OK;
}

int topo_debug_cull_pairs(topo_ctx* ctx, uint32_t out[2]) {
    TOPO_GUARD(ctx);
    if (!out) return TOPO_ERR_INVALID;
    ctx->r->last_cull_pairs(out);
    return TOPO_OK;
}

int topo_get_timings(topo_ctx* ctx, float out_ms[TOPO_TIMING_SLOTS]) {
    TOPO_GUARD(ctx);
    TOPO_CALL(ctx->r->get_timings(out_ms));
}

int topo_pin_host_buffer(topo_ctx* ctx, void* buffer, size_t bytes) {
    TOPO_GUARD(ctx);
    TOPO_CALL(ctx->r->pin_host_buffer(buffer, bytes));
}

int topo_unpin_host_buffer(topo_ctx* ctx, void* buffer) {
    TOPO_GUARD(ctx);
    TOPO_CALL(ctx->r->unpin_host_buffer(buffer));
}

int topo_get_timing_history(topo_ctx* ctx, uint32_t n_frames, float* out_ms, uint32_t* n_out) {
    TOPO_GUARD(ctx);
    if (!n_out) return TOPO_ERR_INVALID;
    TOPO_CALL(ctx->r->get_timing_history(n_frames, out_ms, n_out));
}

int topo_set_timing_slots(topo_ctx* ctx, uint32_t slot_mask) {
    TOPO_GUARD(ctx);
    TOPO_CALL(ctx->r->set_timing_slots(slot_mask));
}

int topo_set_occlusion_split(topo_ctx* ctx, float metres) {
    TOPO_GUARD(ctx);
    return ctx->r->set_occlusion_split(metres);
}

int topo_get_counters(topo_ctx* ctx, uint32_t out[6]) {
    TOPO_GUARD(ctx);
    TOPO_CALL(ctx->r->get_counters(out));
}

int topo_read_normals(topo_ctx* ctx, int32_t lat, int32_t lon, uint8_t* out) {
    TOPO_GUARD(ctx);
    TOPO_CALL(ctx->r->read_normals(lat, lon, out));
}

int topo_read_tile_tables(topo_ctx* ctx, int32_t lat, int32_t lon, float* minmax_out, float* trig_out, double* bounds_out, uint32_t* n_blocks_out) {
    TOPO_GUARD(ctx);
    TOPO_CALL(ctx->r->read_tile_tables(lat, lon, minmax_out, trig_out, bounds_out, n_blocks_out));
}

int topo_visible_peaks(topo_ctx* ctx, uint32_t n_peaks, const float* peaks_xyz, uint8_t* visible_out, uint32_t* xy_out) {
    TOPO_GUARD(ctx);
    TOPO_CALL(ctx->r->visible_peaks(n_peaks, peaks_xyz, visible_out, xy_out));
}

int topo_visible_peaks_device(topo_ctx* ctx, const topo_uniforms* view, uint32_t width, uint32_t height, const float* depth_dev,
                              size_t depth_pitch, uint32_t n_peaks, const float* peaks_xyz_dev, uint8_t* visible_dev,
                              uint32_t* xy_dev) {
    TOPO_GUARD(ctx);
    TOPO_CALL(ctx->r->visible_peaks_device(view, width, height, depth_dev, depth_pitch, n_peaks, peaks_xyz_dev, visible_dev, xy_dev));
}

int topo_probe_sincos(topo_ctx* ctx, const float* x, float* s, float* c, size_t n) {
    TOPO_GUARD(ctx);
    TOPO_CALL(ctx->r->probe_sincos(x, s, c, n));
}

int topo_set_pipeline_depth(topo_ctx* ctx, int32_t depth) {
    TOPO_GUARD(ctx);
    TOPO_CALL(ctx->r->set_pipeline_depth(depth));
}

int topo_join(topo_ctx* ctx) {
    TOPO_GUARD(ctx);
    TOPO_CALL(ctx->r->join_frames());
}

struct topo_comm {
    topo::Comm* c = nullptr;
};

int topo_comm_unique_id(uint8_t out_id[TOPO_COMM_ID_BYTES]) {
    if (!out_id) return TOPO_ERR_INVALID;
    try {
        return topo::comm_unique_id(out_id, &g_create_error);
    } catch (const std::exception& e) {
        g_create_error = e.what();
// ... 335 lines not shown
```

topo-renderer_amd/csrc/topo_kernels.h:

```cpp
#pragma once

#include <hip/hip_runtime.h>
#include <hip/hip_ext.h>

#include "topo_pipeline.h"
#include "topo_ground.h"
#include "topo_unwrap.h"
#include "topo_los.h"

namespace topo {

constexpr uint32_t kBCX = 60, kBCY = 15;
constexpr uint32_t kVX = kBCX + 1, kVY = kBCY + 1;
#ifndef TOPO_RESOLVE_RPW
#define TOPO_RESOLVE_RPW 8
#endif
constexpr uint32_t kResolveBlockW = 64, kResolveBlockH = 4 * TOPO_RESOLVE_RPW;

struct WorkItem {
    uint32_t view_rank;
    uint32_t block;
};

struct FarItem {
    uint32_t view_rank;
    uint32_t block;
    uint16_t x0, x1, y0, y1;
    uint32_t zmin_bits;
};

struct BigItem {
    uint32_t view;
    uint32_t id;
    uint32_t region;
    int32_t X[3], Y[3];
    float z[3];
};

struct RareItem {
    uint32_t view;
    uint32_t draw;
};

struct FrameParams {
    const TileDev* tiles;
    const ViewDev* views;
    uint64_t* vis;
    uint8_t* dirty;
    WorkItem* work;
    uint32_t* counters;
    uint32_t* status_out;
    BigItem* big;
    RareItem* rare;
    FarItem* far;
    WorkItem* work2;
    uint32_t work_cap, big_cap, rare_cap;
    uint32_t far_sub_cap;
    uint32_t near_cap;
    uint32_t near_strip;
    float split_m;
    uint32_t n_views, n_tiles;
    int32_t W, H;
    uint32_t tile_w, tile_h;
    uint32_t bx_count, by_count;
    uint32_t tris_per_tile;
    FastDiv div_tris, div_hm1;
    uint32_t sky_c8;
    uint32_t linear_target;
    uint32_t bgra;
    uint32_t rblocks_x, rblocks_view;
    uint32_t post_off;
    uint32_t rblock_first, rblock_count;
    FastDiv div_rblocks_x, div_rblocks_view;
};

struct OutputParams {
    uint8_t* rgba;
    size_t rgba_view_stride, rgba_pitch;
    float* depth;
    size_t depth_view_stride, depth_pitch;
};

constexpr uint32_t kStatusBigOverflow = 1u;
constexpr uint32_t kStatusRareOverflow = 2u;
constexpr uint32_t kFarLists = 64;
constexpr uint32_t kStatusWords = 16;
constexpr uint32_t kCounterWords = kStatusWords + 16 * kFarLists;
constexpr uint32_t kStatusBounds = 4u;
constexpr uint32_t kCtrWork = 0, kCtrBig = 1;
constexpr uint32_t kCtrStatus = 2;
constexpr uint32_t kCtrRare = 3;
constexpr uint32_t kCtrFarTested = 4, kCtrFarSurvived = 5;
constexpr uint32_t kCtrBigStart = 6, kCtrRareStart = 7;
constexpr uint32_t kCtrBoundsTag = 8, kCtrBoundsLo = 9, kCtrBoundsHi = 10;
constexpr uint32_t far_list_counter(uint32_t q) { return kStatusWords + 16 * q; }

struct EdgeJob {
    uint32_t lt, rb;
    uint32_t uni;
    uint32_t top_bottom;
};
struct CornerJob {
    uint32_t lt, rt, lb, rb;
    uint32_t uni;
};

void launch_block_tables(const TileDev* tiles, uint32_t first, uint32_t count, uint32_t w, uint32_t h, hipStream_t s);
bool normals_tables_fused(uint32_t w, uint32_t h, int lds_rows);
void launch_trig_tables(const TileDev* tiles, uint32_t first, uint32_t count, uint32_t w, uint32_t h, hipStream_t s);
void launch_normals_tables(const TileDev* tiles, uint32_t first, uint32_t count, uint32_t w, uint32_t h, hipStream_t s);
void launch_block_bounds(const TileDev* tiles, uint32_t first, uint32_t count, uint32_t w, uint32_t h, hipStream_t s);
void launch_normals_interior(const TileDev* tiles, uint32_t first, uint32_t count, uint32_t w, uint32_t h, int lds_rows,
                             hipStream_t s);
void launch_normals_border(const TileDev* tiles, const EdgeJob* edges, uint32_t n_edges, const CornerJob* corners, uint32_t n_corners, uint32_t w,
                           uint32_t h, hipStream_t s);

constexpr uint32_t kPackViews = 8;
struct ViewPack { ViewDev v[kPackViews]; };
void launch_put_views(const ViewPack& pack, uint32_t n, ViewDev* dst, hipStream_t s);
constexpr uint32_t kMaxCullPairs = 1024;
void launch_clear(const FrameParams& p, uint32_t* zero, hipStream_t s, hipEvent_t start = nullptr);
void launch_clear_cull(const FrameParams& p, uint32_t* zero, hipStream_t s, hipEvent_t start = nullptr, const ViewPack* pack = nullptr, uint32_t n_pack_views = 0,
                       const uint16_t* pairs = nullptr, uint32_t n_pairs = 0);
void launch_cull(const FrameParams& p, hipStream_t s, const uint16_t* pairs = nullptr, uint32_t n_pairs = 0);
size_t cull_workgroups_max(uint32_t n_views, uint32_t n_tiles, uint32_t blocks_per_tile);
void launch_raster(const FrameParams& p, int phase, hipStream_t s);
void launch_occlusion(const FrameParams& p, hipStream_t s);
void launch_raster_rare(const FrameParams& p, hipStream_t s);
void launch_raster_big(const FrameParams& p, hipStream_t s);
void launch_resolve(const FrameParams& p, const OutputParams& o, hipStream_t s, hipEvent_t start = nullptr, hipEvent_t stop = nullptr);

constexpr uint32_t kViewshedStatSlots = 1024;
void launch_viewshed(const FrameParams& p, uint32_t* const* masks, unsigned long long* stats, hipStream_t s);

struct HorizonPoint {
    int32_t row;
    float depth;
    int32_t lat, lon;
    uint32_t cell_x, cell_y, fan, reserved;
};
struct HorizonParams {
    const uint64_t* vis;
    const uint8_t* dirty;
    const uint32_t* counters;
    uint32_t* check;
    const int32_t* tile_ll;
    HorizonPoint* out;
    size_t view_stride;
    size_t n_keys;
    uint32_t first_view, n_views;
    uint32_t W, H;
    uint32_t n_tiles, tris_per_tile, hm1;
    FastDiv div_tris, div_hm1;
};
void launch_horizon(const HorizonParams& p, hipStream_t s);

struct GroundPoint {
    double lon_deg, lat_deg;
    float height_m, range_m, depth;
    int32_t kind;
    int32_t tile_lat, tile_lon;
    uint32_t cell_x, cell_y, tri, fan;
    float w1, w2;
};
struct GroundQuery { uint32_t view, x, y, reserved; };
struct GroundParams {
    HorizonParams q;
    const TileDev* tiles;
    const GroundView* views;
    const double* trig;
    size_t trig_doubles;
    uint32_t tile_w, tile_h;
    uint32_t sub_views;
};
void launch_ground_tables(const TileDev* tiles, uint32_t n_tiles, double* trig, uint32_t w, uint32_t h, hipStream_t s);
void launch_ground(const GroundParams& p, const GroundQuery* queries, GroundPoint* out, uint32_t n, hipStream_t s);
void launch_ground_map(const GroundParams& p, float* out, size_t view_stride, size_t pitch, hipStream_t s);

static_assert(kLosBCX == kBCX && kLosBCY == kBCY, "topo_los.h walks the raster blocks");
struct RayHit {
    double t, lon_deg, lat_deg;
    float height_m;
    int32_t kind;
    int32_t tile_lat, tile_lon;
    uint32_t cell_x, cell_y, tri, front;
    float w1, w2;
};
struct RayParams {
    LosScene s;
    const int32_t* tile_ll;
    uint32_t* check;
};
void launch_raycast(const RayParams& p, const LosRay* rays, RayHit* out, uint32_t n, hipStream_t s);
void launch_sunlit_map(const GroundParams& g, const LosScene& scene, const double sun[3], uint8_t* out, size_t view_stride, size_t pitch, hipStream_t s);

struct UnwrapParams {
    const double* tab;
    const uint8_t* rgba_src;
    size_t rgba_view_stride, rgba_pitch;
    const uint8_t* depth_src;
    size_t depth_view_stride, depth_pitch;
    uint8_t* rgba_out;
    size_t rgba_out_pitch;
    uint8_t* depth_out;
    size_t depth_out_pitch;
    uint8_t* src_out;
    size_t src_out_pitch;
    uint32_t* check;
    uint32_t n_views, src_w, src_h, out_w, out_h;
    uint32_t blocks_x;
    uint32_t srgb;
};
// ... 25 lines not shown
```

topo-renderer_amd/csrc/topo_kernels.hip:

```cpp
#include <algorithm>
#include <atomic>
#include <cstring>

#include "kernels_common.h"
#include "kernels_load.h"
#include "kernels_frame.h"
#include "kernels_resolve.h"
#include "kernels_query.h"
#include "kernels_overlay.h"
#include "kernels_tiff.h"

namespace topo {


template <typename K, typename... Args>
static inline void launch_timed(K kernel, dim3 grid, dim3 block, hipStream_t s, hipEvent_t start, hipEvent_t stop, const Args&... args) {
    if (start || stop) hipExtLaunchKernelGGL(kernel, grid, block, 0, s, start, stop, 0, args...);
    else hipLaunchKernelGGL(kernel, grid, block, 0, s, args...);
}

struct BlockGrid { uint32_t bxc, byc; };
static inline BlockGrid block_grid(uint32_t w, uint32_t h) { return {(w - 1 + kBCX - 1) / kBCX, (h - 1 + kBCY - 1) / kBCY}; }

template <int kSite, typename K>
// ... 64 lines not shown
        }
#undef TOPO_ROLL
        return;
    }
#define TOPO_K1(R)                                                                                                                    \
    hipLaunchKernelGGL(k_normals_interior<R>, dim3(((((w + 127) / 128) * ((h + (R)-1) / (R)) * count + 7) / 8) * 8), block, 0, s, tiles, first, \
                       count, (int)w, (int)h)
    switch (lds_rows) {
        case 4: TOPO_K1(4); break;
        case 8: TOPO_K1(8); break;
        case 16: TOPO_K1(16); break;
        case 64: TOPO_K1(64); break;
        default: TOPO_K1(32); break;
    }
#undef TOPO_K1
}

void launch_normals_border(const TileDev* tiles, const EdgeJob* edges, uint32_t n_edges, const CornerJob* corners, uint32_t n_corners, uint32_t w,
                           uint32_t h, hipStream_t s) {
    const uint32_t chunks = (w + 63) / 64, blocks = chunks * n_edges + (n_corners + 63) / 64;
    if (blocks == 0) return;
    hipLaunchKernelGGL(k_normals_border, dim3(blocks), dim3(64), 0, s, tiles, edges, n_edges, chunks, corners, n_corners, (int)w, (int)h);
}

void launch_clear(const FrameParams& p, uint32_t* zero, hipStream_t s, hipEvent_t start) {
    const size_t n = (size_t)p.n_views * p.W * p.H;
    launch_timed(k_clear, dim3(2048), dim3(256), s, start, nullptr, p.vis, p.dirty, n, p.counters, zero);
}
void launch_put_views(const ViewPack& pack, uint32_t n, ViewDev* dst, hipStream_t s) {
    hipLaunchKernelGGL(k_put_views, dim3(1), dim3(256), 0, s, pack, n * (uint32_t)(sizeof(ViewDev) / 4), (uint32_t*)dst);
}

namespace {
struct CullGrid {
    unsigned n_blocks;
    uint32_t wgs_per_pair;
    CullPairs list{};
    CullGrid(const FrameParams& p, const uint16_t* pairs, uint32_t n_pairs) {
        const uint32_t blocks_per_tile = p.bx_count * p.by_count;
        if (pairs && n_pairs <= kMaxCullPairs && blocks_per_tile) {
            wgs_per_pair = (blocks_per_tile + 255) / 256;
            n_blocks = n_pairs * wgs_per_pair;
            memcpy(list.code, pairs, n_pairs * sizeof(uint16_t));
        } else {
            wgs_per_pair = 0;
            n_blocks = (unsigned)(((size_t)p.n_views * p.n_tiles * blocks_per_tile + 255) / 256);
        }
    }
};
}
size_t cull_workgroups_max(uint32_t n_views, uint32_t n_tiles, uint32_t blocks_per_tile) {
    const size_t pairs = (size_t)n_views * n_tiles;
    return std::max((pairs * blocks_per_tile + 255) / 256, pairs * ((blocks_per_tile + 255) / 256));
}

void launch_clear_cull(const FrameParams& p, uint32_t* zero, hipStream_t s, hipEvent_t start, const ViewPack* pack, uint32_t n_pack_views, const uint16_t* pairs,
                       uint32_t n_pairs) {
    const CullGrid g(p, pairs, n_pairs);
    const unsigned n_clear = 2048;
    static const ViewPack none{};
    const ViewPack& pk = pack ? *pack : none;
    const uint32_t words = pack ? n_pack_views * (uint32_t)(sizeof(ViewDev) / 4) : 0u;
    launch_timed(k_clear_cull, dim3(g.n_blocks + n_clear), dim3(256), s, start, nullptr, p, g.n_blocks, n_clear, zero, pk, words, g.wgs_per_pair, g.list);
}

void launch_cull(const FrameParams& p, hipStream_t s, const uint16_t* pairs, uint32_t n_pairs) {
    const CullGrid g(p, pairs, n_pairs);
    if (g.n_blocks == 0) return;
    hipLaunchKernelGGL(k_cull, dim3(g.n_blocks), dim3(256), 0, s, p, g.wgs_per_pair, g.list);
}

void launch_raster(const FrameParams& p, int phase, hipStream_t s) {
    if (p.n_tiles == 0) return;
    const unsigned grid = resident_grid<0>(k_raster, 256 * 5);
    hipLaunchKernelGGL(k_raster, dim3(grid), dim3(256), 0, s, p, phase);
}

void launch_occlusion(const FrameParams& p, hipStream_t s) {
    if (p.n_tiles == 0) return;
    const unsigned grid = resident_grid<1>(k_occlusion, 256 * 8);
    hipLaunchKernelGGL(k_occlusion, dim3(grid), dim3(256), 0, s, p);
}

void launch_raster_rare(const FrameParams& p, hipStream_t s) {
    if (p.n_tiles == 0) return;
    hipLaunchKernelGGL(k_raster_rare, dim3(256), dim3(256), 0, s, p);
}

void launch_raster_big(const FrameParams& p, hipStream_t s) {
    if (p.n_tiles == 0) return;
    const unsigned grid = resident_grid<2>(k_raster_big, 256 * 4);
    hipLaunchKernelGGL(k_raster_big, dim3(grid), dim3(256), 0, s, p);
}

void launch_resolve(const FrameParams& p, const OutputParams& o, hipStream_t s, hipEvent_t start, hipEvent_t stop) {
    const unsigned n_blocks = p.rblock_count;
    if (n_blocks == 0) return;
    unsigned resident = 4u * resident_grid<3>(k_resolve<true, false>, 256 * TOPO_RESOLVE_WGS);
    if (const char* e = getenv("TOPO_RESOLVE_GRID")) resident = (unsigned)atoi(e) ? (unsigned)atoi(e) : n_blocks;
    const dim3 grid(n_blocks < resident ? n_blocks : resident), block(256);
    const bool bgra = p.bgra && !p.post_off;
    auto launch = [&](auto kernel) { launch_timed(kernel, grid, block, s, start, stop, p, o); };
    if (!p.linear_target && !bgra) launch(k_resolve<true, false>);
    else if (!p.linear_target) launch(k_resolve<true, true>);
    else if (!bgra) launch(k_resolve<false, false>);
    else launch(k_resolve<false, true>);
}

void launch_viewshed(const FrameParams& p, uint32_t* const* masks, unsigned long long* stats, hipStream_t s) {
    if (p.n_tiles == 0) return;
    const size_t groups = (((size_t)p.n_views * p.W * p.H + 63) / 64 + 63) / 64;
    const unsigned grid = (unsigned)((groups + 3) / 4 < kViewshedStatSlots ? (groups + 3) / 4 : kViewshedStatSlots);
    hipLaunchKernelGGL(k_viewshed, dim3(grid), dim3(256), 0, s, p, masks, stats);
}

void launch_horizon(const HorizonParams& p, hipStream_t s) {
    const uint64_t waves = (uint64_t)((p.W + 63) / 64) * p.n_views;
    if (waves == 0) return;
    hipLaunchKernelGGL(k_horizon, dim3((unsigned)((waves + 3) / 4)), dim3(256), 0, s, p);
}

void launch_ground_tables(const TileDev* tiles, uint32_t n_tiles, double* trig, uint32_t w, uint32_t h, hipStream_t s) {
    if (n_tiles == 0) return;
    hipLaunchKernelGGL(k_ground_tables, dim3((w + h + 255) / 256, n_tiles), dim3(256), 0, s, tiles, trig, w, h);
}

void launch_ground(const GroundParams& p, const GroundQuery* queries, GroundPoint* out, uint32_t n, hipStream_t s) {
    if (n == 0) return;
    hipLaunchKernelGGL(k_ground, dim3((n + 255) / 256), dim3(256), 0, s, p, queries, out, n);
}

void launch_ground_map(const GroundParams& p, float* out, size_t view_stride, size_t pitch, hipStream_t s) {
    const uint64_t view_keys = (uint64_t)p.q.W * p.q.H, k0 = p.q.first_view * view_keys, k1 = k0 + p.q.n_views * view_keys;
    if (k1 == k0) return;
    const uint64_t waves = ((k1 + 63) >> 6) - (k0 >> 6);
    const uint64_t blocks = (waves + 3) / 4;
    hipLaunchKernelGGL(k_ground_map, dim3((unsigned)(blocks < (1u << 20) ? blocks : (1u << 20))), dim3(256), 0, s, p, (uint8_t*)out, view_stride, pitch);
}

void launch_unwrap(const UnwrapParams& p, bool bilinear, hipStream_t s, hipEvent_t start, hipEvent_t stop) {
    UnwrapParams q = p;
    q.blocks_x = (p.out_w + 255) / 256;
    const uint64_t blocks = (uint64_t)q.blocks_x * ((p.out_h + 3) / 4);
    if (blocks == 0 || blocks > 0x7FFFFFFFull) return;
    if (bilinear) launch_timed(k_unwrap<true>, dim3((unsigned)blocks), dim3(256), s, start, stop, q);
    else launch_timed(k_unwrap<false>, dim3((unsigned)blocks), dim3(256), s, start, stop, q);
}

static void overlay_keys_init(uint64_t* keys, int32_t W, int32_t H, bool keys_fresh, hipStream_t s) {
    const size_t n = (size_t)W * H;
    if (keys_fresh) hipLaunchKernelGGL(k_overlay_init, dim3((unsigned)((n + 255) / 256)), dim3(256), 0, s, keys, n);
}

void launch_overlay(const OverlayVertex* verts, const uint32_t* idx, uint32_t n_tris, uint32_t n_verts, float width, int32_t W, int32_t H, uint64_t* keys,
                    bool keys_fresh, uint8_t* rgba, size_t pitch, uint32_t linear_target, uint32_t bgra, hipStream_t s) {
    overlay_keys_init(keys, W, H, keys_fresh, s);
    if (n_tris == 0) return;
    hipLaunchKernelGGL(k_overlay_raster, dim3((n_tris + 63) / 64), dim3(64), 0, s, verts, idx, n_tris, n_verts, width, W, H, keys);
    hipLaunchKernelGGL(k_overlay_resolve, dim3((W + 63) / 64, (H + 3) / 4), dim3(256), 0, s, verts, idx, width, W, H, keys, rgba, pitch, linear_target, bgra);
}

void launch_overlay_glyphs(const GlyphInstance* glyphs, uint32_t n_glyphs, float depth, const uint8_t* atlas, uint32_t aw, uint32_t ah, int32_t W, int32_t H,
                           uint64_t* keys, bool keys_fresh, uint8_t* rgba, size_t pitch, uint32_t linear_target, uint32_t bgra, hipStream_t s) {
    overlay_keys_init(keys, W, H, keys_fresh, s);
    if (n_glyphs == 0) return;
    hipLaunchKernelGGL(k_glyph_raster, dim3(n_glyphs), dim3(64), 0, s, glyphs, n_glyphs, depth, W, H, keys);
    hipLaunchKernelGGL(k_glyph_resolve, dim3(n_glyphs), dim3(64), 0, s, glyphs, n_glyphs, depth, atlas, aw, ah, W, H, keys, rgba, pitch, linear_target, bgra);
}

void launch_post_pixelize(uint32_t n_views, int32_t W, int32_t H, float vw, float vh, float pixelize_n, const uint8_t* pre_rgba, const OutputParams& out,
                          const float* depth, size_t depth_view_stride, size_t depth_pitch, uint32_t linear_target, uint32_t bgra, hipStream_t s) {
    hipLaunchKernelGGL(k_post_pixelize, dim3((W + 63) / 64, (H + 3) / 4, n_views), dim3(256), 0, s, W, H, vw, vh, pixelize_n, pre_rgba, out, depth, depth_view_stride,
                       depth_pitch, linear_target, bgra);
}

// ... 22 lines not shown
```

topo-renderer_amd/csrc/topo_pipeline.h:

```cpp
#pragma once

#include "topo_math.h"

namespace topo {

struct TileDev {
    const float* heights;
    uint32_t* normals;
    const float* block_minmax;
    const float* trig_lon;
    const float* trig_lat;
    const double* block_bounds;
    float raster_x, raster_y;
    float model_x, model_y;
    float scale_x, scale_y;
    float rot[9];
    float pad_;
};

struct ViewDev {
    float proj[16];
    float cam_x, cam_y;
    float sun[3];
    int32_t view_mode;
// ... 226 lines not shown
        if (!dead) {
            int32_t F0 = r0 + m0 * lo, F1 = r1 + m1 * lo, F2 = r2 + m2 * lo;
            for (int32_t k = lo; k <= hi; ++k) {
                if ((F0 | F1 | F2) >= 0) {
                    const float w1 = (float)(F1 - b1) * iA, w2 = (float)(F2 - b2) * iA;
                    float z = fmaf(w1, dz1, fmaf(w2, dz2, z0));
                    if (z < 1.0f) {
                        if (z < 0.0f) z = 0.0f;
                        emit((uint32_t)py * (uint32_t)W + (uint32_t)(px0 + k), vis_key(z, id));
                    }
                }
                F0 += m0;
                F1 += m1;
                F2 += m2;
            }
        }
        r0 -= dx0 * 256;
        r1 -= dx1 * 256;
        r2 -= dx2 * 256;
    }
}

template <typename Emit4>
TOPO_HD void big_medium_lane(const int32_t X[3], const int32_t Y[3], const float zv[3], uint32_t id, int32_t W, int32_t H,
                             int32_t rx, int32_t ry, uint32_t lane, Emit4&& emit4) {
    const int32_t X0 = X[0], Y0 = Y[0], X1 = X[1], Y1 = Y[1], X2 = X[2], Y2 = Y[2];
    const int32_t mnx = X0 < X1 ? (X0 < X2 ? X0 : X2) : (X1 < X2 ? X1 : X2), mxx = X0 > X1 ? (X0 > X2 ? X0 : X2) : (X1 > X2 ? X1 : X2);
    const int32_t mny = Y0 < Y1 ? (Y0 < Y2 ? Y0 : Y2) : (Y1 < Y2 ? Y1 : Y2), mxy = Y0 > Y1 ? (Y0 > Y2 ? Y0 : Y2) : (Y1 > Y2 ? Y1 : Y2);
    const int32_t area2 = (X1 - X0) * (Y2 - Y0) - (Y1 - Y0) * (X2 - X0);
    if (area2 >= 0) return;
    int32_t px0 = (mnx + 127) >> 8, px1 = (mxx - 128) >> 8, py0 = (mny + 127) >> 8, py1 = (mxy - 128) >> 8;
    px0 = px0 > 0 ? px0 : 0; px1 = px1 < W - 1 ? px1 : W - 1;
    py0 = py0 > 0 ? py0 : 0; py1 = py1 < H - 1 ? py1 : H - 1;
    px0 = px0 > rx * 64 ? px0 : rx * 64; px1 = px1 < rx * 64 + 63 ? px1 : rx * 64 + 63;
    py0 = py0 > ry * 64 ? py0 : ry * 64; py1 = py1 < ry * 64 + 63 ? py1 : ry * 64 + 63;
    const int32_t bw = px1 - px0 + 1, bh = py1 - py0 + 1;
    if (bw <= 0 || bh <= 0) return;
    const int32_t dx0 = X2 - X1, dy0 = Y2 - Y1, dx1 = X0 - X2, dy1 = Y0 - Y2, dx2 = X1 - X0, dy2 = Y1 - Y0;
    const int32_t b0 = ((dy0 > 0) || (dy0 == 0 && dx0 < 0)) ? 0 : -1;
    const int32_t b1 = ((dy1 > 0) || (dy1 == 0 && dx1 < 0)) ? 0 : -1;
    const int32_t b2 = ((dy2 > 0) || (dy2 == 0 && dx2 < 0)) ? 0 : -1;
    const int32_t cx0 = px0 * 256 + 128, cy0 = py0 * 256 + 128;
    const int32_t R0 = dy0 * (cx0 - X1) - dx0 * (cy0 - Y1) + b0;
    const int32_t R1 = dy1 * (cx0 - X2) - dx1 * (cy0 - Y2) + b1;
    const int32_t R2 = dy2 * (cx0 - X0) - dx2 * (cy0 - Y0) + b2;
    const int32_t A0 = dy0 * 256, A1 = dy1 * 256, A2 = dy2 * 256, B0 = dx0 * 256, B1 = dx1 * 256, B2 = dx2 * 256;
    const float iA = div_f(1.0f, (float)(-area2));
    const float z0 = zv[0], dz1 = zv[1] - zv[0], dz2 = zv[2] - zv[0];
    const uint32_t sh = bw <= 8 ? 3u : bw <= 16 ? 4u : bw <= 32 ? 5u : 6u;
    const int32_t u = (int32_t)(lane & ((1u << sh) - 1u)), v0 = (int32_t)(lane >> sh), rows = 64 >> sh;
    int32_t F0 = R0 + TOPO_MUL24(A0, u) - TOPO_MUL24(B0, v0);
    int32_t F1 = R1 + TOPO_MUL24(A1, u) - TOPO_MUL24(B1, v0);
    int32_t F2 = R2 + TOPO_MUL24(A2, u) - TOPO_MUL24(B2, v0);
    const int32_t S0 = B0 * rows, S1 = B1 * rows, S2 = B2 * rows;
    uint32_t pixel = (uint32_t)(py0 + v0) * (uint32_t)W + (uint32_t)(px0 + u);
    const uint32_t pstep = (uint32_t)(rows * W);
    const bool ucol = u < bw;
    int32_t yrow = py0 + v0;
    for (int32_t vb = 0; vb < bh; vb += 4 * rows) {
        uint32_t pix[4];
        uint64_t key[4];
        int32_t pyk[4];
#pragma unroll
        for (int k = 0; k < 4; ++k) {
            key[k] = kVisClear;
            pix[k] = pixel;
            pyk[k] = yrow;
            if (ucol && vb + k * rows + v0 < bh && (F0 | F1 | F2) >= 0) {
                const float w1 = (float)(F1 - b1) * iA, w2 = (float)(F2 - b2) * iA;
                float z = fmaf(w1, dz1, fmaf(w2, dz2, z0));
                if (z < 1.0f) {
                    if (z < 0.0f) z = 0.0f;
                    key[k] = vis_key(z, id);
                }
            }
            F0 -= S0; F1 -= S1; F2 -= S2;
            pixel += pstep;
            yrow += rows;
        }
        emit4(pix, key, pyk);
    }
}

template <typename Emit>
TOPO_HD void big_giant_lane(const int32_t X[3], const int32_t Y[3], const float zv[3], uint32_t id, int32_t W, int32_t H,
                            int32_t rx, int32_t ry, uint32_t lane, Emit&& emit) {
    SVert s[3];
#pragma unroll
    for (int k = 0; k < 3; ++k) { s[k].X = X[k]; s[k].Y = Y[k]; s[k].z = zv[k]; s[k].flag = kVtxOk; }
    TriSetup ts;
    if (!triangle_setup(s[0], s[1], s[2], W, H, ts)) return;
    const int32_t bx0 = ts.px0 > rx * 64 ? ts.px0 : rx * 64, bx1 = ts.px1 < rx * 64 + 63 ? ts.px1 : rx * 64 + 63;
    const int32_t by0 = ts.py0 > ry * 64 ? ts.py0 : ry * 64, by1 = ts.py1 < ry * 64 + 63 ? ts.py1 : ry * 64 + 63;
    if (bx0 > bx1 || by0 > by1) return;
    const int32_t lx = (int32_t)(lane & 7), ly = (int32_t)(lane >> 3);
    const int32_t sx0 = bx0 & ~7, sy0 = by0 & ~7;
    const int64_t cx = (int64_t)(sx0 + lx) * 256 + 128, cy = (int64_t)(sy0 + ly) * 256 + 128;
    int64_t Fr0 = ts.dy[0] * (cx - ts.ax[0]) - ts.dx[0] * (cy - ts.ay[0]) + ts.bias[0];
    int64_t Fr1 = ts.dy[1] * (cx - ts.ax[1]) - ts.dx[1] * (cy - ts.ay[1]) + ts.bias[1];
    int64_t Fr2 = ts.dy[2] * (cx - ts.ax[2]) - ts.dx[2] * (cy - ts.ay[2]) + ts.bias[2];
    const int64_t ax0 = ts.dy[0] * 2048, ax1 = ts.dy[1] * 2048, ax2 = ts.dy[2] * 2048;
    const int64_t ay0 = ts.dx[0] * 2048, ay1 = ts.dx[1] * 2048, ay2 = ts.dx[2] * 2048;
    const bool narrow = -((X[1] - (int64_t)X[0]) * (Y[2] - (int64_t)Y[0]) - (Y[1] - (int64_t)Y[0]) * (X[2] - (int64_t)X[0])) < (1ll << 48);
    const int32_t b1 = (int32_t)ts.bias[1], b2 = (int32_t)ts.bias[2];
    for (int32_t sy = sy0; sy <= by1; sy += 8) {
        int64_t F0 = Fr0, F1 = Fr1, F2 = Fr2;
        const int32_t py = sy + ly;
        const bool rowin = py >= by0 && py <= by1;
        for (int32_t sx = sx0; sx <= bx1; sx += 8) {
            const int32_t px = sx + lx;
            if (rowin && px >= bx0 && px <= bx1 && (F0 | F1 | F2) >= 0) {
                const int64_t U1 = F1 - b1, U2 = F2 - b2;
                float f1, f2;
                if (narrow) {
                    f1 = fmaf((float)(int32_t)(U1 >> 24), 16777216.0f, (float)(int32_t)((uint32_t)U1 & 0xFFFFFFu));
                    f2 = fmaf((float)(int32_t)(U2 >> 24), 16777216.0f, (float)(int32_t)((uint32_t)U2 & 0xFFFFFFu));
                } else {
                    f1 = (float)U1;
                    f2 = (float)U2;
                }
                float z = fmaf(f1 * ts.iA, ts.dz1, fmaf(f2 * ts.iA, ts.dz2, ts.z0));
                if (z < 1.0f) {
                    if (z < 0.0f) z = 0.0f;
                    emit((size_t)py * W + px, vis_key(z, id), py);
                }
            }
            F0 += ax0; F1 += ax1; F2 += ax2;
        }
        Fr0 -= ay0; Fr1 -= ay1; Fr2 -= ay2;
    }
}

TOPO_HD VFull lerp_vertex(const VFull& I, const VFull& O, float t) {
    VFull r;
#pragma unroll
    for (int k = 0; k < 4; ++k) r.clip[k] = I.clip[k] + t * (O.clip[k] - I.clip[k]);
    r.clip[2] = 0.0f;
    r.wpos = {I.wpos.x + (O.wpos.x - I.wpos.x) * t, I.wpos.y + (O.wpos.y - I.wpos.y) * t,
              I.wpos.z + (O.wpos.z - I.wpos.z) * t};
    r.wnrm = {I.wnrm.x + (O.wnrm.x - I.wnrm.x) * t, I.wnrm.y + (O.wnrm.y - I.wnrm.y) * t,
              I.wnrm.z + (O.wnrm.z - I.wnrm.z) * t};
    return r;
}

TOPO_HD VFull clip_edge(const VFull& I, const VFull& O) {
    return lerp_vertex(I, O, div_wide(I.clip[2], I.clip[2] - O.clip[2]));
}

TOPO_HD bool clip_near_fan(const VFull& v0, const VFull& v1, const VFull& v2, uint32_t fan, VFull& a, VFull& b, VFull& c) {
    const uint32_t mask = (v0.clip[2] >= 0.0f ? 1u : 0u) | (v1.clip[2] >= 0.0f ? 2u : 0u) | (v2.clip[2] >= 0.0f ? 4u : 0u);
    switch (mask) {
        case 7u:
            if (fan != 0) return false;
            a = v0; b = v1; c = v2;
            return true;
        case 1u:
            if (fan != 0) return false;
            a = v0; b = clip_edge(v0, v1); c = clip_edge(v0, v2);
            return true;
        case 2u:
            if (fan != 0) return false;
            a = clip_edge(v1, v0); b = v1; c = clip_edge(v1, v2);
            return true;
        case 4u:
            if (fan != 0) return false;
            a = clip_edge(v2, v1); b = v2; c = clip_edge(v2, v0);
            return true;
        case 3u:
            a = v0;
            if (fan == 0) { b = v1; c = clip_edge(v1, v2); } else { b = clip_edge(v1, v2); c = clip_edge(v0, v2); }
            return fan < 2;
        case 6u:
            a = clip_edge(v1, v0);
            if (fan == 0) { b = v1; c = v2; } else { b = v2; c = clip_edge(v2, v0); }
            return fan < 2;
        case 5u:
            a = v0;
            if (fan == 0) { b = clip_edge(v0, v1); c = clip_edge(v2, v1); } else { b = clip_edge(v2, v1); c = v2; }
            return fan < 2;
        default:
            return false;
    }
}
TOPO_HD bool clip_near_rest(const VFull& v0, const VFull& v1, const VFull& v2, uint32_t fan, float rest[4]) {
    const uint32_t mask = (v0.clip[2] >= 0.0f ? 1u : 0u) | (v1.clip[2] >= 0.0f ? 2u : 0u) | (v2.clip[2] >= 0.0f ? 4u : 0u);
    VFull d;
    switch (mask) {
        case 3u: d = fan == 0 ? clip_edge(v0, v2) : v1; break;
        case 6u: d = fan == 0 ? clip_edge(v2, v0) : v1; break;
        case 5u: d = fan == 0 ? v2 : clip_edge(v0, v1); break;
        default: return false;
    }
#pragma unroll
    for (int k = 0; k < 4; ++k) rest[k] = d.clip[k];
    return true;
}

TOPO_HD void interpolate_q(const VFull& v0, const VFull& v1, const VFull& v2, float q0, float q1, float q2, f3& wpos, f3& wnrm) {
    const float iq = div_f(1.0f, (q0 + q1) + q2);
    wpos.x = fmaf(v2.wpos.x, q2, fmaf(v1.wpos.x, q1, v0.wpos.x * q0)) * iq;
    wpos.y = fmaf(v2.wpos.y, q2, fmaf(v1.wpos.y, q1, v0.wpos.y * q0)) * iq;
    wpos.z = fmaf(v2.wpos.z, q2, fmaf(v1.wpos.z, q1, v0.wpos.z * q0)) * iq;
    wnrm.x = fmaf(v2.wnrm.x, q2, fmaf(v1.wnrm.x, q1, v0.wnrm.x * q0)) * iq;
    wnrm.y = fmaf(v2.wnrm.y, q2, fmaf(v1.wnrm.y, q1, v0.wnrm.y * q0)) * iq;
    wnrm.z = fmaf(v2.wnrm.z, q2, fmaf(v1.wnrm.z, q1, v0.wnrm.z * q0)) * iq;
}
TOPO_HD void recip_w3(float w0, float w1, float w2, float& i0, float& i1, float& i2) {
#if defined(__HIP_DEVICE_COMPILE__)
    if (__builtin_expect(!(fmaxf(fmaxf(w0, w1), w2) <= 0x1p+96f), 0)) {
        i0 = 1.0f / w0; i1 = 1.0f / w1; i2 = 1.0f / w2;
        return;
    }
// ... 326 lines not shown
```

Before: 88600 Mpix/s.

## Add cover pass where one fully covering big triangle owns each 64x64 region

Big triangles that fully cover a 64x64 screen region now claim that region through an atomicMax on a per-region owner word tagged with a frame serial. A new k_raster_cover kernel then rasterizes each region's winning triangle directly, using plain loads and stores on the visibility buffer in place of atomic min per pixel. k_raster_big skips the items that won, which removes the per-pixel edge tests and atomics for them. It is enabled by default for outputs above 32M pixels, which includes the 16384x4096 panorama, but only in the near phase. The cost is one extra kernel launch with a grid of one block per region, plus atomics on the owner array.

```diff
diff --git a/topo-renderer_amd/__init__.py b/topo-renderer_amd/__init__.py
--- a/topo-renderer_amd/__init__.py
+++ b/topo-renderer_amd/__init__.py
@@ -94,6 +94,7 @@
             "topo_debug_far_phase_launched": (C.c_int, [vp, vp]),
             "topo_debug_set_tile_prefilter": (C.c_int, [vp, i32]),
             "topo_debug_cull_pairs": (C.c_int, [vp, vp]),
+            "topo_debug_cover_stats": (C.c_int, [vp, vp]),
             "topo_pin_host_buffer": (C.c_int, [vp, vp, sz]),
             "topo_unpin_host_buffer": (C.c_int, [vp, vp]),
             "topo_get_timings": (C.c_int, [vp, vp]),
@@ -565,6 +566,11 @@
         self._check(lib().topo_debug_cull_pairs(self._h, _p(out)))
         return int(out[0]), int(out[1])
 
+    def debug_cover_stats(self) -> dict:
+        out = np.zeros(3, np.uint32)
+        self._check(lib().topo_debug_cover_stats(self._h, _p(out)))
+        return {"candidates": int(out[0]), "won": int(out[1]), "lost": int(out[2])}
+
     def timings(self) -> dict:
         out = np.zeros(TIMING_SLOTS, np.float32)
         self._check(lib().topo_get_timings(self._h, _p(out)))
diff --git a/topo-renderer_amd/csrc/kernels_frame.h b/topo-renderer_amd/csrc/kernels_frame.h
--- a/topo-renderer_amd/csrc/kernels_frame.h
+++ b/topo-renderer_amd/csrc/kernels_frame.h
@@ -278,8 +278,22 @@
         }
 }
 
-__device__ bool enqueue_big(const FrameParams& P, uint32_t view, uint32_t id, const SVert& s0, const SVert& s1, const SVert& s2,
-                            int32_t px0, int32_t px1, int32_t py0, int32_t py1) {
+__device__ __forceinline__ uint32_t cover_region_index(const CoverParams& C, uint32_t view, int32_t rx, int32_t ry) {
+    return (view * C.regions_y + (uint32_t)ry) * C.regions_x + (uint32_t)rx;
+}
+__device__ __forceinline__ uint64_t cover_bid(const CoverParams& C, uint32_t big_index) { return ((uint64_t)C.serial << 32) | big_index; }
+__device__ __forceinline__ bool cover_claim(const FrameParams& P, const CoverParams& C, const TriSetup& ts, uint32_t view, int32_t rx, int32_t ry,
+                                            uint32_t big_index) {
+    if (!setup_covers_region(ts, P.W, P.H, rx, ry)) return false;
+    const uint32_t r = cover_region_index(C, view, rx, ry);
+    if (!TOPO_CHK(P.counters, view < P.n_views && (uint32_t)rx < C.regions_x && (uint32_t)ry < C.regions_y && r < C.cap, 30u, r)) return false;
+    atomicMax(reinterpret_cast<unsigned long long*>(C.owner + r), (unsigned long long)cover_bid(C, big_index));
+    return true;
+}
+
+template <typename ViewOf>
+__device__ __forceinline__ bool enqueue_big_items(const FrameParams& P, uint32_t view, uint32_t id, const SVert& s0, const SVert& s1, const SVert& s2,
+                                                  int32_t px0, int32_t px1, int32_t py0, int32_t py1, ViewOf&& view_of) {
     const int32_t rx0 = px0 >> 6, rx1 = px1 >> 6, ry0 = py0 >> 6, ry1 = py1 >> 6;
     const uint32_t n = (uint32_t)((rx1 - rx0 + 1) * (ry1 - ry0 + 1));
     const uint32_t base = atomicAdd(&P.counters[kCtrBig], n);
@@ -300,10 +314,23 @@
     for (int32_t ry = ry0; ry <= ry1; ++ry)
         for (int32_t rx = rx0; rx <= rx1; ++rx) {
             it.region = ((uint32_t)ry << 16) | (uint32_t)rx;
-            if (TOPO_CHK(P.counters, k < P.big_cap && rx >= 0 && ry >= 0 && rx * 64 < P.W && ry * 64 < P.H, 7u, k)) P.big[k] = it;
+            if (TOPO_CHK(P.counters, k < P.big_cap && rx >= 0 && ry >= 0 && rx * 64 < P.W && ry * 64 < P.H, 7u, k)) {
+                it.view = view_of(rx, ry, k);
+                P.big[k] = it;
+            }
             ++k;
         }
     return true;
+}
+__device__ bool enqueue_big(const FrameParams& P, uint32_t view, uint32_t id, const SVert& s0, const SVert& s1, const SVert& s2,
+                            int32_t px0, int32_t px1, int32_t py0, int32_t py1) {
+    return enqueue_big_items(P, view, id, s0, s1, s2, px0, px1, py0, py1, [&](int32_t, int32_t, uint32_t) { return view; });
+}
+__device__ bool enqueue_big_cover(const FrameParams& P, const CoverParams& C, const TriSetup& ts, uint32_t view, uint32_t id, const SVert& s0, const SVert& s1,
+                                  const SVert& s2) {
+    return enqueue_big_items(P, view, id, s0, s1, s2, ts.px0, ts.px1, ts.py0, ts.py1, [&](int32_t rx, int32_t ry, uint32_t k) {
+        return C.serial && cover_claim(P, C, ts, view, rx, ry, k) ? view | kBigCovered : view;
+    });
 }
 
 __device__ __forceinline__ void enqueue_rare(const FrameParams& P, uint32_t view, uint32_t draw) {
@@ -517,7 +544,7 @@
 }
 
 constexpr uint32_t kCoopRegions = 24;
-__global__ __launch_bounds__(256) void k_raster_rare(FrameParams P) {
+__global__ __launch_bounds__(256) void k_raster_rare(FrameParams P, CoverParams C) {
     uint32_t count = P.counters[kCtrRare];
     if (count > P.rare_cap) count = P.rare_cap;
     const uint32_t lane = threadIdx.x & 63;
@@ -537,7 +564,7 @@
             const uint32_t rw = (uint32_t)(rx1 - rx0 + 1), n_regions = rw * (uint32_t)(ry1 - ry0 + 1);
             const bool coop = has && !small && n_regions >= kCoopRegions && rw <= 256u;
             bool in_lane = has && small;
-            if (has && !small && !coop) in_lane = !enqueue_big(P, ri.view, id, r.s[0], r.s[1], r.s[2], ts.px0, ts.px1, ts.py0, ts.py1);
+            if (has && !small && !coop) in_lane = !enqueue_big_cover(P, C, ts, ri.view, id, r.s[0], r.s[1], r.s[2]);
             uint64_t jobs = __ballot(coop);
             if (jobs) {
                 const uint64_t act = __ballot(true);
@@ -567,12 +594,24 @@
                         for (uint32_t k = mine; k < n && base + k < P.big_cap; k += n_act) P.big[base + k] = it;
                         continue;
                     }
+                    TriSetup jts;
+                    bool jcover = false;
+                    if (C.serial) {
+                        SVert q[3];
+#pragma unroll
+                        for (int k = 0; k < 3; ++k) { q[k].X = it.X[k]; q[k].Y = it.Y[k]; q[k].z = it.z[k]; q[k].flag = kVtxOk; }
+                        jcover = triangle_setup(q[0], q[1], q[2], P.W, P.H, jts);
+                    }
+                    const uint32_t jview = it.view;
                     const uint32_t magic = region_split_magic(jw);
                     for (uint32_t k = mine; k < n; k += n_act) {
                         const uint32_t q = region_split_row(k, jw, n, magic);
                         const int32_t ry = jy0 + (int32_t)q, rx = jx0 + (int32_t)(k - q * jw);
                         it.region = ((uint32_t)ry << 16) | (uint32_t)rx;
-                        if (TOPO_CHK(P.counters, base + k < P.big_cap && rx >= 0 && ry >= 0 && rx * 64 < P.W && ry * 64 < P.H, 7u, base + k)) P.big[base + k] = it;
+                        if (TOPO_CHK(P.counters, base + k < P.big_cap && rx >= 0 && ry >= 0 && rx * 64 < P.W && ry * 64 < P.H, 7u, base + k)) {
+                            it.view = jcover && cover_claim(P, C, jts, jview, rx, ry, base + k) ? jview | kBigCovered : jview;
+                            P.big[base + k] = it;
+                        }
                     }
                 }
             }
@@ -581,7 +620,63 @@
     }
 }
 
-__global__ __launch_bounds__(256) void k_raster_big(FrameParams P) {
+constexpr int kCoverRows = 16;
+__global__ __launch_bounds__(256) void k_raster_cover(FrameParams P, CoverParams C) {
+    const uint32_t lane = threadIdx.x & 63, wave = __builtin_amdgcn_readfirstlane(threadIdx.x >> 6);
+    const size_t view_keys = (size_t)P.W * P.H, nseg = ((size_t)P.n_views * view_keys + 63) >> 6;
+    (void)nseg;
+    const uint32_t region = blockIdx.x;
+    const uint64_t word = *const_space(C.owner + region);
+    for (bool won = (uint32_t)(word >> 32) == C.serial; won; won = false) {
+        const uint32_t item = (uint32_t)word;
+        if (!TOPO_CHK(P.counters, region < C.cap && item < P.big_cap, 32u, item)) continue;
+        BigItem bi;
+        {
+            const BigItem& g = P.big[item];
+            bi.view = wave_first(g.view); bi.id = wave_first(g.id); bi.region = wave_first(g.region);
+#pragma unroll
+            for (int k = 0; k < 3; ++k) { bi.X[k] = wave_first(g.X[k]); bi.Y[k] = wave_first(g.Y[k]); bi.z[k] = wave_first(g.z[k]); }
+        }
+        const uint32_t view = bi.view & ~kBigCovered;
+        const int32_t rx = (int32_t)(bi.region & 0xFFFFu), ry = (int32_t)(bi.region >> 16);
+        if (!TOPO_CHK(P.counters, (bi.view & kBigCovered) && bi.id != kNoTri && view < P.n_views && rx * 64 < P.W && ry * 64 < P.H &&
+                                      cover_region_index(C, view, rx, ry) == region, 33u, bi.region)) continue;
+        SVert s[3];
+#pragma unroll
+        for (int k = 0; k < 3; ++k) { s[k].X = bi.X[k]; s[k].Y = bi.Y[k]; s[k].z = bi.z[k]; s[k].flag = kVtxOk; }
+        TriSetup ts;
+        if (!triangle_setup(s[0], s[1], s[2], P.W, P.H, ts)) continue;
+        const bool narrow = giant_narrow(bi.X, bi.Y);
+        const Vis vis = view_vis(P, view);
+        const int32_t row0 = (int32_t)wave * kCoverRows, y0 = ry * 64 + row0, x0 = rx * 64, x1 = min(x0 + 63, P.W - 1);
+        if (y0 >= P.H) continue;
+        const bool row = lane < (uint32_t)kCoverRows && y0 + (int32_t)lane < P.H;
+        const size_t first = (size_t)(vis.p - vis.base) + (size_t)(y0 + (int32_t)(row ? lane : 0u)) * P.W;
+        const size_t s0 = (first + x0) >> 6, s1 = (first + x1) >> 6;
+        const bool row_ok = row && TOPO_CHK(P.counters, s1 < nseg, 34u, s1);
+        const bool marked = row_ok && (vis.dirty[s0] | vis.dirty[s1]) != 0;
+        const uint32_t marked_rows = (uint32_t)__ballot(marked);
+        const int32_t px = x0 + (int32_t)lane;
+        uint64_t old[kCoverRows];
+#pragma unroll
+        for (int j = 0; j < kCoverRows; ++j) {
+            old[j] = kVisClear;
+            if ((marked_rows >> j & 1u) && px < P.W) {
+                const size_t pix = (size_t)(y0 + j) * P.W + px;
+                if (TOPO_CHK(P.counters, y0 + j < P.H && pix < view_keys, 35u, pix)) old[j] = vis.p[pix];
+            }
+        }
+        big_cover_lane<kCoverRows>(ts, narrow, bi.id, P.W, P.H, rx, ry, row0, lane, [&](size_t pix, uint64_t key, int j) {
+            if (TOPO_CHK(P.counters, pix < view_keys, 36u, pix)) vis.p[pix] = key < old[j] ? key : old[j];
+        });
+        if (row_ok) {
+            vis.dirty[s0] = 1;
+            if (s1 != s0) vis.dirty[s1] = 1;
+        }
+    }
+}
+
+__global__ __launch_bounds__(256) void k_raster_big(FrameParams P, CoverParams C) {
     __shared__ uint8_t s_rows[4][64];
     uint32_t count = P.counters[kCtrBig];
     if (count > P.big_cap) count = P.big_cap;
@@ -597,8 +692,15 @@
             for (int k = 0; k < 3; ++k) { bi.X[k] = wave_first(g.X[k]); bi.Y[k] = wave_first(g.Y[k]); bi.z[k] = wave_first(g.z[k]); }
         }
         if (bi.id == kNoTri) continue;
+        const int32_t rx = (int32_t)(bi.region & 0xFFFFu), ry = (int32_t)(bi.region >> 16);
+        if (bi.view & kBigCovered) {
+            bi.view &= ~kBigCovered;
+            const uint32_t r = cover_region_index(C, bi.view, rx, ry);
+            if (C.serial != 0u && TOPO_CHK(P.counters, bi.view < P.n_views && rx * 64 < P.W && ry * 64 < P.H && r < C.cap, 31u, r) &&
+                *const_space(C.owner + r) == cover_bid(C, item))
+                continue;
+        }
         const Vis vis = view_vis(P, bi.view);
-        const int32_t rx = (int32_t)(bi.region & 0xFFFFu), ry = (int32_t)(bi.region >> 16);
         if (!TOPO_CHK(P.counters, bi.view < P.n_views && rx * 64 < P.W && ry * 64 < P.H, 11u, bi.region)) continue;
         uint8_t* const rows = s_rows[wave];
         if (spans_fit_int32(bi.X[0], bi.Y[0], bi.X[1], bi.Y[1], bi.X[2], bi.Y[2])) {
diff --git a/topo-renderer_amd/csrc/terrain_renderer.cpp b/topo-renderer_amd/csrc/terrain_renderer.cpp
--- a/topo-renderer_amd/csrc/terrain_renderer.cpp
+++ b/topo-renderer_amd/csrc/terrain_renderer.cpp
@@ -23,6 +23,7 @@
     const bool fuse_clear_cull = env("TOPO_FUSE_CLEAR_CULL", 1) != 0;
     const bool tile_prefilter = env("TOPO_TILE_PREFILTER", 1) != 0;
     const int near_strip = env("TOPO_NEAR_STRIP", 0);
+    const int cover = env("TOPO_COVER", -1);
 };
 const Switches& switches() { static const Switches s; return s; }
 
@@ -511,6 +512,20 @@
     if (int rc = ensure(stream, c.d_far, (far_sub_cap ? far_sub_cap * kFarLists : 1) * sizeof(FarItem))) return rc;
     if (int rc = ensure(stream, c.d_big, p.big_cap * sizeof(BigItem))) return rc;
     if (int rc = ensure(stream, c.d_rare, p.rare_cap * sizeof(RareItem))) return rc;
+    c.cover = CoverParams{};
+    constexpr size_t kCoverMinPixels = (size_t)1 << 25;
+    if (p.n_tiles && (switches().cover > 0 || (switches().cover < 0 && pixels > kCoverMinPixels))) {
+        const uint32_t regions_x = (w + 63) / 64, regions_y = (h + 63) / 64;
+        const size_t regions = (size_t)n * regions_x * regions_y;
+        const bool fresh = regions * sizeof(uint64_t) > c.d_cover.cap;
+        if (int rc = ensure(stream, c.d_cover, regions * sizeof(uint64_t))) return rc;
+        if (fresh || c.cover_serial == 0xFFFFFFFFu) {
+            TOPO_HIP_TRY(hipMemsetAsync(c.d_cover.p, 0, c.d_cover.cap, stream));
+            c.cover_serial = 0;
+        }
+        c.cover = CoverParams{c.d_cover.as<uint64_t>(), ++c.cover_serial, (uint32_t)regions, regions_x, regions_y};
+        c.cover_big_cap = p.big_cap;
+    }
     if (!c.d_counters.p) {
         if (int rc = ensure(stream, c.d_counters, 2 * kCounterWords * sizeof(uint32_t))) return rc;
         TOPO_HIP_TRY(hipMemsetAsync(c.d_counters.p, 0, 2 * kCounterWords * sizeof(uint32_t), stream));
@@ -625,16 +640,17 @@
     TOPO_HIP_TRY(mark(kStRasterNear));
     launch_raster(p, 0, stream);
     TOPO_HIP_TRY(mark(kStRareBigNear));
-    launch_raster_rare(p, stream);
-    launch_raster_big(p, stream);
+    launch_raster_rare(p, c.cover, stream);
+    launch_raster_cover(p, c.cover, stream);
+    launch_raster_big(p, c.cover, stream);
     TOPO_HIP_TRY(mark(kStOcclusion));
     if (far_phase) launch_occlusion(p, stream);
     TOPO_HIP_TRY(mark(kStRasterFar));
     if (far_phase) launch_raster(p, 1, stream);
     TOPO_HIP_TRY(mark(kStRareBigFar));
     if (far_phase) {
-        launch_raster_rare(p, stream);
-        launch_raster_big(p, stream);
+        launch_raster_rare(p, CoverParams{}, stream);
+        launch_raster_big(p, CoverParams{}, stream);
     }
     TOPO_HIP_TRY(mark(kStResolve, true));
     const hipEvent_t ev_rstart = own(kStResolve), ev_rstop = own(kNumStages);
@@ -1027,6 +1043,25 @@
     return TOPO_OK;
 }
 
+int TerrainRenderer::cover_stats(uint32_t out[3]) {
+    out[0] = out[1] = out[2] = 0;
+    FrameCtx& fc = ctx_[last_ctx_];
+    if (!fc.h_status.p || !fc.submitted) return TOPO_OK;
+    if (int rc = bind_device()) return rc;
+    if (fc.last_stream) TOPO_HIP_TRY(hipStreamSynchronize(fc.last_stream));
+    const CoverParams& cv = fc.cover;
+    if (!cv.serial) return TOPO_OK;
+    const uint32_t n_big = std::min(fc.latest_status()[kCtrBig], fc.cover_big_cap);
+    std::vector<BigItem> items(n_big);
+    std::vector<uint64_t> owner(cv.cap);
+    if (n_big) TOPO_HIP_TRY(hipMemcpy(items.data(), fc.d_big.p, n_big * sizeof(BigItem), hipMemcpyDeviceToHost));
+    if (cv.cap) TOPO_HIP_TRY(hipMemcpy(owner.data(), cv.owner, cv.cap * sizeof(uint64_t), hipMemcpyDeviceToHost));
+    for (const BigItem& it : items) out[0] += it.id != kNoTri && (it.view & kBigCovered) ? 1u : 0u;
+    for (uint64_t w : owner) out[1] += (uint32_t)(w >> 32) == cv.serial ? 1u : 0u;
+    out[2] = out[0] - out[1];
+    return TOPO_OK;
+}
+
 int TerrainRenderer::read_normals(int32_t lat, int32_t lon, uint8_t* out) {
     Tile* t = find(lat, lon);
     if (!t) return fail(TOPO_ERR_NOT_FOUND, "no such tile");
diff --git a/topo-renderer_amd/csrc/terrain_renderer.hpp b/topo-renderer_amd/csrc/terrain_renderer.hpp
--- a/topo-renderer_amd/csrc/terrain_renderer.hpp
+++ b/topo-renderer_amd/csrc/terrain_renderer.hpp
@@ -118,6 +118,7 @@
     int get_timings(float out[TOPO_TIMING_SLOTS]);
     int get_timing_history(uint32_t n_frames, float* out_ms, uint32_t* n_out);
     int get_counters(uint32_t out[6]);
+    int cover_stats(uint32_t out[3]);
     int frame_status(uint32_t out[4]);
     int set_occlusion_split(float metres);
     int set_timing_slots(uint32_t mask);
@@ -219,6 +220,10 @@
         const uint32_t* latest_status() const { return status_words(submitted - 1); }
         DeviceBuffer d_vis, d_dirty;
         DeviceBuffer d_work, d_work2, d_far, d_big, d_rare, d_counters;
+        DeviceBuffer d_cover;
+        uint32_t cover_serial = 0;
+        CoverParams cover{};
+        uint32_t cover_big_cap = 0;
         DeviceBuffer d_pre_rgba, d_pre_depth;
         struct Submission {
             uint32_t n_views = 0;
diff --git a/topo-renderer_amd/csrc/topo_capi.cpp b/topo-renderer_amd/csrc/topo_capi.cpp
--- a/topo-renderer_amd/csrc/topo_capi.cpp
+++ b/topo-renderer_amd/csrc/topo_capi.cpp
@@ -146,6 +146,12 @@
     return TOPO_OK;
 }
 
+int topo_debug_cover_stats(topo_ctx* ctx, uint32_t out[3]) {
+    TOPO_GUARD(ctx);
+    if (!out) return TOPO_ERR_INVALID;
+    TOPO_CALL(ctx->r->cover_stats(out));
+}
+
 int topo_get_timings(topo_ctx* ctx, float out_ms[TOPO_TIMING_SLOTS]) {
     TOPO_GUARD(ctx);
     TOPO_CALL(ctx->r->get_timings(out_ms));
diff --git a/topo-renderer_amd/csrc/topo_kernels.h b/topo-renderer_amd/csrc/topo_kernels.h
--- a/topo-renderer_amd/csrc/topo_kernels.h
+++ b/topo-renderer_amd/csrc/topo_kernels.h
@@ -74,6 +74,13 @@
     FastDiv div_rblocks_x, div_rblocks_view;
 };
 
+struct CoverParams {
+    uint64_t* owner;
+    uint32_t serial;
+    uint32_t cap;
+    uint32_t regions_x, regions_y;
+};
+
 struct OutputParams {
     uint8_t* rgba;
     size_t rgba_view_stride, rgba_pitch;
@@ -86,6 +93,7 @@
 constexpr uint32_t kFarLists = 64;
 constexpr uint32_t kStatusWords = 16;
 constexpr uint32_t kCounterWords = kStatusWords + 16 * kFarLists;
+constexpr uint32_t kBigCovered = 0x80000000u;
 constexpr uint32_t kStatusBounds = 4u;
 constexpr uint32_t kCtrWork = 0, kCtrBig = 1;
 constexpr uint32_t kCtrStatus = 2;
@@ -126,8 +134,9 @@
 size_t cull_workgroups_max(uint32_t n_views, uint32_t n_tiles, uint32_t blocks_per_tile);
 void launch_raster(const FrameParams& p, int phase, hipStream_t s);
 void launch_occlusion(const FrameParams& p, hipStream_t s);
-void launch_raster_rare(const FrameParams& p, hipStream_t s);
-void launch_raster_big(const FrameParams& p, hipStream_t s);
+void launch_raster_rare(const FrameParams& p, const CoverParams& cover, hipStream_t s);
+void launch_raster_cover(const FrameParams& p, const CoverParams& cover, hipStream_t s);
+void launch_raster_big(const FrameParams& p, const CoverParams& cover, hipStream_t s);
 void launch_resolve(const FrameParams& p, const OutputParams& o, hipStream_t s, hipEvent_t start = nullptr, hipEvent_t stop = nullptr);
 
 constexpr uint32_t kViewshedStatSlots = 1024;
diff --git a/topo-renderer_amd/csrc/topo_kernels.hip b/topo-renderer_amd/csrc/topo_kernels.hip
--- a/topo-renderer_amd/csrc/topo_kernels.hip
+++ b/topo-renderer_amd/csrc/topo_kernels.hip
@@ -170,15 +170,20 @@
     hipLaunchKernelGGL(k_occlusion, dim3(grid), dim3(256), 0, s, p);
 }
 
-void launch_raster_rare(const FrameParams& p, hipStream_t s) {
-    if (p.n_tiles == 0) return;
-    hipLaunchKernelGGL(k_raster_rare, dim3(256), dim3(256), 0, s, p);
-}
-
-void launch_raster_big(const FrameParams& p, hipStream_t s) {
+void launch_raster_rare(const FrameParams& p, const CoverParams& cover, hipStream_t s) {
+    if (p.n_tiles == 0) return;
+    hipLaunchKernelGGL(k_raster_rare, dim3(256), dim3(256), 0, s, p, cover);
+}
+
+void launch_raster_cover(const FrameParams& p, const CoverParams& cover, hipStream_t s) {
+    if (p.n_tiles == 0 || cover.serial == 0 || cover.cap == 0) return;
+    hipLaunchKernelGGL(k_raster_cover, dim3(cover.cap), dim3(256), 0, s, p, cover);
+}
+
+void launch_raster_big(const FrameParams& p, const CoverParams& cover, hipStream_t s) {
     if (p.n_tiles == 0) return;
     const unsigned grid = resident_grid<2>(k_raster_big, 256 * 4);
-    hipLaunchKernelGGL(k_raster_big, dim3(grid), dim3(256), 0, s, p);
+    hipLaunchKernelGGL(k_raster_big, dim3(grid), dim3(256), 0, s, p, cover);
 }
 
 void launch_resolve(const FrameParams& p, const OutputParams& o, hipStream_t s, hipEvent_t start, hipEvent_t stop) {
diff --git a/topo-renderer_amd/csrc/topo_pipeline.h b/topo-renderer_amd/csrc/topo_pipeline.h
--- a/topo-renderer_amd/csrc/topo_pipeline.h
+++ b/topo-renderer_amd/csrc/topo_pipeline.h
@@ -332,6 +332,25 @@
     }
 }
 
+TOPO_HD bool giant_narrow(const int32_t X[3], const int32_t Y[3]) {
+    return -((X[1] - (int64_t)X[0]) * (Y[2] - (int64_t)Y[0]) - (Y[1] - (int64_t)Y[0]) * (X[2] - (int64_t)X[0])) < (1ll << 48);
+}
+TOPO_HD bool giant_depth(const TriSetup& ts, bool narrow, int64_t U1, int64_t U2, float& z) {
+    float f1, f2;
+    if (narrow) {
+        f1 = fmaf((float)(int32_t)(U1 >> 24), 16777216.0f, (float)(int32_t)((uint32_t)U1 & 0xFFFFFFu));
+        f2 = fmaf((float)(int32_t)(U2 >> 24), 16777216.0f, (float)(int32_t)((uint32_t)U2 & 0xFFFFFFu));
+    } else {
+        f1 = (float)U1;
+        f2 = (float)U2;
+    }
+    float zz = fmaf(f1 * ts.iA, ts.dz1, fmaf(f2 * ts.iA, ts.dz2, ts.z0));
+    if (!(zz < 1.0f)) return false;
+    if (zz < 0.0f) zz = 0.0f;
+    z = zz;
+    return true;
+}
+
 template <typename Emit>
 TOPO_HD void big_giant_lane(const int32_t X[3], const int32_t Y[3], const float zv[3], uint32_t id, int32_t W, int32_t H,
                             int32_t rx, int32_t ry, uint32_t lane, Emit&& emit) {
@@ -351,7 +370,7 @@
     int64_t Fr2 = ts.dy[2] * (cx - ts.ax[2]) - ts.dx[2] * (cy - ts.ay[2]) + ts.bias[2];
     const int64_t ax0 = ts.dy[0] * 2048, ax1 = ts.dy[1] * 2048, ax2 = ts.dy[2] * 2048;
     const int64_t ay0 = ts.dx[0] * 2048, ay1 = ts.dx[1] * 2048, ay2 = ts.dx[2] * 2048;
-    const bool narrow = -((X[1] - (int64_t)X[0]) * (Y[2] - (int64_t)Y[0]) - (Y[1] - (int64_t)Y[0]) * (X[2] - (int64_t)X[0])) < (1ll << 48);
+    const bool narrow = giant_narrow(X, Y);
     const int32_t b1 = (int32_t)ts.bias[1], b2 = (int32_t)ts.bias[2];
     for (int32_t sy = sy0; sy <= by1; sy += 8) {
         int64_t F0 = Fr0, F1 = Fr1, F2 = Fr2;
@@ -360,24 +379,54 @@
         for (int32_t sx = sx0; sx <= bx1; sx += 8) {
             const int32_t px = sx + lx;
             if (rowin && px >= bx0 && px <= bx1 && (F0 | F1 | F2) >= 0) {
-                const int64_t U1 = F1 - b1, U2 = F2 - b2;
-                float f1, f2;
-                if (narrow) {
-                    f1 = fmaf((float)(int32_t)(U1 >> 24), 16777216.0f, (float)(int32_t)((uint32_t)U1 & 0xFFFFFFu));
-                    f2 = fmaf((float)(int32_t)(U2 >> 24), 16777216.0f, (float)(int32_t)((uint32_t)U2 & 0xFFFFFFu));
-                } else {
-                    f1 = (float)U1;
-                    f2 = (float)U2;
-                }
-                float z = fmaf(f1 * ts.iA, ts.dz1, fmaf(f2 * ts.iA, ts.dz2, ts.z0));
-                if (z < 1.0f) {
-                    if (z < 0.0f) z = 0.0f;
-                    emit((size_t)py * W + px, vis_key(z, id), py);
-                }
+                float z;
+                if (giant_depth(ts, narrow, F1 - b1, F2 - b2, z)) emit((size_t)py * W + px, vis_key(z, id), py);
             }
             F0 += ax0; F1 += ax1; F2 += ax2;
         }
         Fr0 -= ay0; Fr1 -= ay1; Fr2 -= ay2;
+    }
+}
+
+TOPO_HD bool setup_covers_region(const TriSetup& ts, int32_t W, int32_t H, int32_t rx, int32_t ry) {
+    const int32_t x0 = rx * 64, y0 = ry * 64;
+    const int32_t x1 = x0 + 63 < W - 1 ? x0 + 63 : W - 1, y1 = y0 + 63 < H - 1 ? y0 + 63 : H - 1;
+    if (rx < 0 || ry < 0 || x0 > x1 || y0 > y1) return false;
+    if (ts.px0 > x0 || ts.px1 < x1 || ts.py0 > y0 || ts.py1 < y1) return false;
+    bool in = true;
+#pragma unroll
+    for (int e = 0; e < 3; ++e) {
+        const int64_t cx = (int64_t)(ts.dy[e] >= 0 ? x0 : x1) * 256 + 128, cy = (int64_t)(ts.dx[e] >= 0 ? y1 : y0) * 256 + 128;
+        in = in && ts.dy[e] * (cx - ts.ax[e]) - ts.dx[e] * (cy - ts.ay[e]) + ts.bias[e] >= 0;
+    }
+    return in;
+}
+TOPO_HD bool item_covers_region(const int32_t X[3], const int32_t Y[3], int32_t W, int32_t H, int32_t rx, int32_t ry) {
+    SVert s[3];
+#pragma unroll
+    for (int k = 0; k < 3; ++k) { s[k].X = X[k]; s[k].Y = Y[k]; s[k].z = 0.0f; s[k].flag = kVtxOk; }
+    TriSetup ts;
+    return triangle_setup(s[0], s[1], s[2], W, H, ts) && setup_covers_region(ts, W, H, rx, ry);
+}
+
+template <int kRows, typename Emit>
+TOPO_HD void big_cover_lane(const TriSetup& ts, bool narrow, uint32_t id, int32_t W, int32_t H, int32_t rx, int32_t ry, int32_t row0,
+                            uint32_t lane, Emit&& emit) {
+    const int32_t px = rx * 64 + (int32_t)lane, py0 = ry * 64 + row0;
+    if (rx < 0 || ry < 0 || row0 < 0 || lane >= 64u || px >= W) return;
+    const int64_t cx = (int64_t)px * 256 + 128, cy = (int64_t)py0 * 256 + 128;
+    int64_t U1 = ts.dy[1] * (cx - ts.ax[1]) - ts.dx[1] * (cy - ts.ay[1]);
+    int64_t U2 = ts.dy[2] * (cx - ts.ax[2]) - ts.dx[2] * (cy - ts.ay[2]);
+    const int64_t s1 = ts.dx[1] * 256, s2 = ts.dx[2] * 256;
+    size_t pix = (size_t)py0 * W + px;
+#pragma unroll
+    for (int j = 0; j < kRows; ++j) {
+        if (py0 + j < H) {
+            float z;
+            if (giant_depth(ts, narrow, U1, U2, z)) emit(pix, vis_key(z, id), j);
+        }
+        U1 -= s1; U2 -= s2;
+        pix += (size_t)W;
     }
 }
 
```

Measured after the change: 94680 Mpix/s, median of 6. 1.07x the previous value.
